# Lornatang/Real_ESRGAN-PyTorch

Measured on NVIDIA B200. Metric: x4 RRDBNet LR Mpix/s, higher is better.
Workload: dtype fp16

## Files before the change

include/resr.h:

```cpp
#ifndef RESR_H_
#define RESR_H_

#include <stddef.h>
#include <stdint.h>

#ifdef __cplusplus
extern "C" {
#endif

#define RESR_OK 0
#define RESR_E_INVALID 1
#define RESR_E_CUDA 2
#define RESR_E_NOMEM 3

int resr_version(void);
const char* resr_last_error(void);

typedef struct resr_generator resr_generator_t;

int resr_generator_create(resr_generator_t** out, int in_channels, int out_channels, int upscale_factor);
void resr_generator_destroy(resr_generator_t* g);

size_t resr_generator_num_params(void);
int resr_generator_num_tensors(void);
int resr_generator_tensor_span(int index, size_t* offset, size_t* count);

int resr_generator_load_params(resr_generator_t* g, const float* flat_params, void* stream);

size_t resr_generator_workspace_bytes(int n, int h, int w);
int resr_generator_set_precision(resr_generator_t* g, int precision);
size_t resr_generator_workspace_bytes_for(const resr_generator_t* g, int n, int h, int w);

int resr_generator_forward(resr_generator_t* g, const float* x, float* y, int n, int h, int w, void* workspace,
                           size_t workspace_bytes, void* stream);

int resr_generator_forward_u8(resr_generator_t* g, const unsigned char* x_u8, unsigned char* y_u8, int n, int h, int w,
                              void* workspace, size_t workspace_bytes, void* stream);
int resr_generator_forward_u8_host(resr_generator_t* g, const unsigned char* x_u8_host, unsigned char* y_u8_host, int n, int h, int w,
                                   void* workspace, size_t workspace_bytes, void* stream);
int resr_tensor_to_image_u8(const float* x, unsigned char* out_hwc, int c, int h, int w, int range_norm, int half, void* stream);

int resr_generator_forward_host(resr_generator_t* g, const float* x_host, float* y_host, int n, int h, int w,
                                void* workspace, size_t workspace_bytes, void* stream);

int resr_generator_forward_host_async(resr_generator_t* g, const float* x_host, float* y_host, int n, int h, int w,
                                      void* workspace, size_t workspace_bytes, void* stream);
int resr_generator_host_sync(resr_generator_t* g);

int resr_generator_launches_per_forward(void);
int resr_set_conv_pair_policy(int policy);
int resr_debug_wait_profile(unsigned long long* out16_host, int reset);

typedef struct resr_conv_desc {
    const void* in16;
    int n, h, w, c_total, cin, cout;
    int fmt_in;
    int mode;
    const float* weight;
    const float* bias;
    int ep_mode;
    int lrelu, clamp01;
    void* out16;
    int out16_fmt, out16_cstride, out16_choff, out16_up2;
    float* outf;
    int outf_cstride, outf_choff;
    const void* res1;
    const void* res2;
    int res_cstride, res_choff;
    int res16, res16_fmt;
    float* out_nchw;
    int out_nchw_c;
    int dbg_flags;
    unsigned long long* dbg;
} resr_conv_desc;
int resr_conv3x3(const resr_conv_desc* d, void* stream);

int resr_nchw_to_nhwc16(const float* x, void* out16, int n, int c, int h, int w, int c_pad, int fmt, void* stream);


int resr_filter2d(const float* image, const float* kernel, float* out, int b, int c, int h, int w, int k,
                  int kernel_batch, void* stream);

size_t resr_usm_workspace_bytes(int b, int c, int h, int w);
int resr_usm_sharp(const float* image, float* out, int b, int c, int h, int w, int radius, int sigma, float weight,
                   float threshold, void* workspace, size_t workspace_bytes, void* stream);
size_t resr_usm_backward_workspace_bytes(int b, int c, int h, int w);
int resr_usm_sharp_backward(const float* image, const float* grad_out, float* grad_in, int b, int c, int h, int w,
                            int radius, int sigma, float weight, float threshold, void* workspace,
                            size_t workspace_bytes, void* stream);

int resr_resize(const float* image, float* out, int planes, int h_in, int w_in, int h_out, int w_out, int mode,
                double scale_h, double scale_w, void* stream);

int resr_gaussian_noise_apply(const float* image, float* out, const float* sigma, const float* gray,
                              const float* noise_color, const float* noise_gray, int b, int c, int h, int w, int clip,
                              int rounds, void* stream);

size_t resr_poisson_workspace_bytes(int b);
int resr_unique_count_u8(const float* image, int* counts_color, int* counts_gray, int b, int c, int h, int w,
                         void* workspace, size_t workspace_bytes, void* stream);
int resr_poisson_rates(const float* image, float* rate_color, float* rate_gray, int b, int c, int h, int w,
                       void* workspace, size_t workspace_bytes, void* stream);
int resr_poisson_noise_apply(const float* image, float* out, const float* scale, const float* gray,
                             const float* samples_color, const float* samples_gray, int b, int c, int h, int w, int clip,
                             int rounds, void* workspace, size_t workspace_bytes, int reuse_counts, void* stream);

int resr_gaussian_noise_sampled(const float* image, float* out, const float* sigma, const float* gray, int b, int c, int h, int w,
                                int clip, int rounds, unsigned long long seed, unsigned long long* call_state, void* stream);

int resr_poisson_noise_sampled(const float* image, float* out, const float* scale, const float* gray, int b, int c, int h, int w,
                               int clip, int rounds, unsigned long long seed, unsigned long long* call_counter,
                               void* workspace, size_t workspace_bytes, void* stream);

int resr_jpeg(const float* image, float* out, const float* quality, float* factor_out, int b, int h, int w,
              int clamp_input, float* q_y, float* q_cb, float* q_cr, void* stream);

int resr_augment_batch_u8(const unsigned char* images_bgr_hwc, float* out_rgb_nchw, const int* ops, int b, int h, int w,
                          void* stream);

int resr_crop(const float* image, float* out, int planes, int h_in, int w_in, int top, int left, int h_out, int w_out,
              int round_to_u8, void* stream);

typedef struct resr_kernel_params {
    int type, kernel_size, isotropic, reserved;
    double sigma_x, sigma_y, theta, beta, cutoff;
} resr_kernel_params;
int resr_synthesize_kernels(const resr_kernel_params* params_host, int count, int pad, double* out_f64, float* out_f32,
                            void* stream);
int resr_synthesize_kernels_device(const resr_kernel_params* params_dev, int count, int kmax, int pad, double* out_f64,
                                   float* out_f32, void* stream);
typedef struct resr_kernel_draw_config {
    int n_sizes, sizes[16];
    int sinc_size_split;
    int final_size;
    double sinc_prob1, sinc_prob2, sinc_prob3;
    double prob1[6], prob2[6];
    double sigma_range1[2], sigma_range2[2];
    double gen_beta_range1[2], gen_beta_range2[2], plateau_beta_range1[2], plateau_beta_range2[2];
} resr_kernel_draw_config;
int resr_draw_degradation_kernel_params(const resr_kernel_draw_config* cfg, int batch, unsigned long long seed,
                                        unsigned long long* call_state, resr_kernel_params* params_dev, void* stream);

size_t resr_generator_train_workspace_bytes(int n, int h, int w);
int resr_generator_forward_train(resr_generator_t* g, const float* x, float* y, int n, int h, int w, void* workspace,
                                 size_t workspace_bytes, void* stream);
int resr_generator_backward_l1(resr_generator_t* g, const float* hr, float* grads_flat, float* loss_out, int n, int h,
                               int w, void* workspace, size_t workspace_bytes, void* stream);
int resr_generator_train_step_l1(resr_generator_t* g, const float* x, const float* hr, float* y, float* grads_flat,
                                 float* loss_out, int n, int h, int w, void* workspace, size_t workspace_bytes,
                                 void* stream);
int resr_generator_step_is_graph(resr_generator_t* g);
int resr_generator_grad_buckets(size_t* offsets, int max_entries);
int resr_generator_wait_grad_bucket(resr_generator_t* g, int bucket, void* stream);
int resr_generator_backward(resr_generator_t* g, const float* dy, float* grads_flat, int n, int h, int w, void* workspace,
                            size_t workspace_bytes, void* stream);

size_t resr_conv3x3_wgrad_workspace_bytes(int n, int h, int w, int cin, int cout);
int resr_conv3x3_wgrad(const void* x16, int x_cstride, int fmt_x, const void* dy16_bf16, int n, int h, int w, int cin,
                       int cout, float* dw, float* db, void* workspace, size_t workspace_bytes, void* stream);

size_t resr_conv3x3_wgrad_nhwc_workspace_bytes(void);
int resr_conv3x3_wgrad_nhwc(const void* x_bf16, int x_cstride, const void* dy_bf16, int dy_cstride, int n, int h, int w,
                            int cin, int cout, float* dw, float* db, void* workspace, size_t workspace_bytes, void* stream);

int resr_niqe_num_blocks(int h, int w, int crop_border, int block);
size_t resr_niqe_workspace_bytes(int b, int h, int w, int crop_border, int block);
int resr_niqe_features(const float* image_rgb, double* features, int b, int h, int w, int crop_border, int block,
                       void* workspace, size_t workspace_bytes, void* stream);

typedef struct resr_resize_spec {
    int mode;
    int out_h, out_w;
    double scale;
} resr_resize_spec;
typedef struct resr_noise_spec {
    int type;
    const float* param;
    const float* gray;
    int gray_any;
    const float* draws_color;
    const float* draws_gray;
    unsigned long long seed;
} resr_noise_spec;
typedef struct resr_degrade_plan {
    int batch, hr_h, hr_w;
    int usm_radius, usm_sigma;
    float usm_weight, usm_threshold;
    int blur1, blur2, final_order;
    int kernel_size, sinc_batched;
    resr_resize_spec resize1, resize2, resize3;
    resr_noise_spec noise1, noise2;
    const float* jpeg1_quality;
    const float* jpeg2_quality;
    int crop_top, crop_left, image_size, upscale;
    unsigned long long* rng_state;
} resr_degrade_plan;
size_t resr_degrade_workspace_bytes(const resr_degrade_plan* plan);
int resr_degrade_batch(const resr_degrade_plan* plan, const float* hr, const float* kernel1, const float* kernel2,
                       const float* sinc_kernel, float* lr_out, float* hr_out, void* workspace, size_t workspace_bytes,
                       void* stream);

int resr_adam_ema_step(float* params, const float* grads, float* exp_avg, float* exp_avg_sq, float* ema_shadow, size_t n,
                       float lr, float beta1, float beta2, float eps, long long step, float ema_decay, float grad_scale,
                       void* stream);

#ifdef __cplusplus
}
#endif
#endif
```

real_esrgan-pytorch_b200/_lib.py:

```python
import ctypes
import os
from ctypes import POINTER, Structure, c_char_p, c_double, c_float, c_int, c_size_t, c_void_p

_HERE = os.path.dirname(os.path.abspath(__file__))
LIB_PATH = os.environ.get("RESR_LIB_PATH") or os.path.join(_HERE, "lib", "libresr.so")


class ResrError(RuntimeError):
    pass


class ConvDesc(Structure):
    _fields_ = [
        ("in16", c_void_p),
        ("n", c_int), ("h", c_int), ("w", c_int), ("c_total", c_int), ("cin", c_int), ("cout", c_int),
        ("fmt_in", c_int), ("mode", c_int),
        ("weight", c_void_p), ("bias", c_void_p),
        ("ep_mode", c_int), ("lrelu", c_int), ("clamp01", c_int),
        ("out16", c_void_p),
        ("out16_fmt", c_int), ("out16_cstride", c_int), ("out16_choff", c_int), ("out16_up2", c_int),
        ("outf", c_void_p),
        ("outf_cstride", c_int), ("outf_choff", c_int),
        ("res1", c_void_p), ("res2", c_void_p),
        ("res_cstride", c_int), ("res_choff", c_int),
        ("res16", c_int), ("res16_fmt", c_int),
        ("out_nchw", c_void_p),
        ("out_nchw_c", c_int),
        ("dbg_flags", c_int),
        ("dbg", c_void_p),
    ]


class ResizeSpec(Structure):
    _fields_ = [("mode", c_int), ("out_h", c_int), ("out_w", c_int), ("scale", c_double)]


class NoiseSpec(Structure):
    _fields_ = [("type", c_int), ("param", c_void_p), ("gray", c_void_p), ("gray_any", c_int), ("draws_color", c_void_p),
                ("draws_gray", c_void_p), ("seed", ctypes.c_ulonglong)]


class DegradePlan(Structure):
    _fields_ = [("batch", c_int), ("hr_h", c_int), ("hr_w", c_int),
                ("usm_radius", c_int), ("usm_sigma", c_int), ("usm_weight", c_float), ("usm_threshold", c_float),
                ("blur1", c_int), ("blur2", c_int), ("final_order", c_int), ("kernel_size", c_int), ("sinc_batched", c_int),
                ("resize1", ResizeSpec), ("resize2", ResizeSpec), ("resize3", ResizeSpec),
                ("noise1", NoiseSpec), ("noise2", NoiseSpec),
                ("jpeg1_quality", c_void_p), ("jpeg2_quality", c_void_p),
                ("crop_top", c_int), ("crop_left", c_int), ("image_size", c_int), ("upscale", c_int),
                ("rng_state", c_void_p)]


class KernelParams(Structure):
    _fields_ = [("type", c_int), ("kernel_size", c_int), ("isotropic", c_int), ("reserved", c_int),
                ("sigma_x", c_double), ("sigma_y", c_double), ("theta", c_double), ("beta", c_double),
                ("cutoff", c_double)]


class KernelDrawConfig(Structure):
    _fields_ = [("n_sizes", c_int), ("sizes", c_int * 16), ("sinc_size_split", c_int), ("final_size", c_int),
                ("sinc_prob1", c_double), ("sinc_prob2", c_double), ("sinc_prob3", c_double),
                ("prob1", c_double * 6), ("prob2", c_double * 6),
                ("sigma_range1", c_double * 2), ("sigma_range2", c_double * 2),
                ("gen_beta_range1", c_double * 2), ("gen_beta_range2", c_double * 2),
                ("plateau_beta_range1", c_double * 2), ("plateau_beta_range2", c_double * 2)]


SIGNATURES = {
    "resr_version": (c_int, []),
    "resr_last_error": (c_char_p, []),
    "resr_generator_create": (c_int, [POINTER(c_void_p), c_int, c_int, c_int]),
    "resr_generator_destroy": (None, [c_void_p]),
    "resr_generator_num_params": (c_size_t, []),
    "resr_generator_num_tensors": (c_int, []),
    "resr_generator_tensor_span": (c_int, [c_int, POINTER(c_size_t), POINTER(c_size_t)]),
    "resr_generator_load_params": (c_int, [c_void_p, c_void_p, c_void_p]),
    "resr_generator_workspace_bytes": (c_size_t, [c_int, c_int, c_int]),
    "resr_generator_workspace_bytes_for": (c_size_t, [c_void_p, c_int, c_int, c_int]),
    "resr_generator_set_precision": (c_int, [c_void_p, c_int]),
    "resr_generator_forward": (c_int, [c_void_p, c_void_p, c_void_p, c_int, c_int, c_int, c_void_p, c_size_t, c_void_p]),
    "resr_generator_forward_u8": (c_int, [c_void_p, c_void_p, c_void_p, c_int, c_int, c_int, c_void_p, c_size_t, c_void_p]),
    "resr_generator_forward_u8_host": (c_int, [c_void_p, c_void_p, c_void_p, c_int, c_int, c_int, c_void_p, c_size_t, c_void_p]),
    "resr_tensor_to_image_u8": (c_int, [c_void_p, c_void_p, c_int, c_int, c_int, c_int, c_int, c_void_p]),
    "resr_generator_forward_host": (c_int, [c_void_p, c_void_p, c_void_p, c_int, c_int, c_int, c_void_p, c_size_t, c_void_p]),
    "resr_generator_forward_host_async": (c_int, [c_void_p, c_void_p, c_void_p, c_int, c_int, c_int, c_void_p, c_size_t, c_void_p]),
    "resr_generator_host_sync": (c_int, [c_void_p]),
    "resr_generator_launches_per_forward": (c_int, []),
    "resr_debug_wait_profile": (c_int, [c_void_p, c_int]),
    "resr_set_conv_pair_policy": (c_int, [c_int]),
    "resr_conv3x3": (c_int, [POINTER(ConvDesc), c_void_p]),
    "resr_nchw_to_nhwc16": (c_int, [c_void_p, c_void_p, c_int, c_int, c_int, c_int, c_int, c_int, c_void_p]),
    "resr_filter2d": (c_int, [c_void_p, c_void_p, c_void_p, c_int, c_int, c_int, c_int, c_int, c_int, c_void_p]),
    "resr_usm_workspace_bytes": (c_size_t, [c_int, c_int, c_int, c_int]),
    "resr_niqe_num_blocks": (c_int, [c_int, c_int, c_int, c_int]),
    "resr_niqe_workspace_bytes": (c_size_t, [c_int, c_int, c_int, c_int, c_int]),
    "resr_niqe_features": (c_int, [c_void_p, c_void_p, c_int, c_int, c_int, c_int, c_int, c_void_p, c_size_t, c_void_p]),
    "resr_augment_batch_u8": (c_int, [c_void_p, c_void_p, c_void_p, c_int, c_int, c_int, c_void_p]),
    "resr_usm_backward_workspace_bytes": (c_size_t, [c_int, c_int, c_int, c_int]),
    "resr_usm_sharp_backward": (c_int, [c_void_p, c_void_p, c_void_p, c_int, c_int, c_int, c_int, c_int, c_int, c_float, c_float,
                                        c_void_p, c_size_t, c_void_p]),
    "resr_usm_sharp": (c_int, [c_void_p, c_void_p, c_int, c_int, c_int, c_int, c_int, c_int, c_float, c_float, c_void_p,
                               c_size_t, c_void_p]),
    "resr_resize": (c_int, [c_void_p, c_void_p, c_int, c_int, c_int, c_int, c_int, c_int, c_double, c_double, c_void_p]),
    "resr_gaussian_noise_apply": (c_int, [c_void_p, c_void_p, c_void_p, c_void_p, c_void_p, c_void_p, c_int, c_int, c_int,
                                          c_int, c_int, c_int, c_void_p]),
    "resr_poisson_workspace_bytes": (c_size_t, [c_int]),
    "resr_unique_count_u8": (c_int, [c_void_p, c_void_p, c_void_p, c_int, c_int, c_int, c_int, c_void_p, c_size_t, c_void_p]),
    "resr_poisson_rates": (c_int, [c_void_p, c_void_p, c_void_p, c_int, c_int, c_int, c_int, c_void_p, c_size_t, c_void_p]),
    "resr_poisson_noise_apply": (c_int, [c_void_p, c_void_p, c_void_p, c_void_p, c_void_p, c_void_p, c_int, c_int, c_int,
                                         c_int, c_int, c_int, c_void_p, c_size_t, c_int, c_void_p]),
    "resr_gaussian_noise_sampled": (c_int, [c_void_p, c_void_p, c_void_p, c_void_p, c_int, c_int, c_int, c_int, c_int, c_int,
                                            ctypes.c_ulonglong, c_void_p, c_void_p]),
    "resr_poisson_noise_sampled": (c_int, [c_void_p, c_void_p, c_void_p, c_void_p, c_int, c_int, c_int, c_int, c_int, c_int,
                                           ctypes.c_ulonglong, c_void_p, c_void_p, c_size_t, c_void_p]),
    "resr_jpeg": (c_int, [c_void_p, c_void_p, c_void_p, c_void_p, c_int, c_int, c_int, c_int, c_void_p, c_void_p, c_void_p,
                          c_void_p]),
    "resr_degrade_workspace_bytes": (c_size_t, [POINTER(DegradePlan)]),
    "resr_degrade_batch": (c_int, [POINTER(DegradePlan), c_void_p, c_void_p, c_void_p, c_void_p, c_void_p, c_void_p, c_void_p,
                                   c_size_t, c_void_p]),
    "resr_adam_ema_step": (c_int, [c_void_p, c_void_p, c_void_p, c_void_p, c_void_p, c_size_t, c_float, c_float, c_float,
                                   c_float, ctypes.c_longlong, c_float, c_float, c_void_p]),
    "resr_synthesize_kernels": (c_int, [POINTER(KernelParams), c_int, c_int, c_void_p, c_void_p, c_void_p]),
    "resr_synthesize_kernels_device": (c_int, [c_void_p, c_int, c_int, c_int, c_void_p, c_void_p, c_void_p]),
    "resr_draw_degradation_kernel_params": (c_int, [POINTER(KernelDrawConfig), c_int, ctypes.c_ulonglong, c_void_p, c_void_p, c_void_p]),
    "resr_generator_train_workspace_bytes": (c_size_t, [c_int, c_int, c_int]),
    "resr_generator_forward_train": (c_int, [c_void_p, c_void_p, c_void_p, c_int, c_int, c_int, c_void_p, c_size_t, c_void_p]),
    "resr_generator_backward_l1": (c_int, [c_void_p, c_void_p, c_void_p, c_void_p, c_int, c_int, c_int, c_void_p, c_size_t,
                                           c_void_p]),
    "resr_generator_train_step_l1": (c_int, [c_void_p, c_void_p, c_void_p, c_void_p, c_void_p, c_void_p, c_int, c_int, c_int,
                                             c_void_p, c_size_t, c_void_p]),
    "resr_generator_step_is_graph": (c_int, [c_void_p]),
    "resr_generator_backward": (c_int, [c_void_p, c_void_p, c_void_p, c_int, c_int, c_int, c_void_p, c_size_t, c_void_p]),
    "resr_conv3x3_wgrad_workspace_bytes": (c_size_t, [c_int, c_int, c_int, c_int, c_int]),
    "resr_generator_grad_buckets": (c_int, [c_void_p, c_int]),
    "resr_generator_wait_grad_bucket": (c_int, [c_void_p, c_int, c_void_p]),
    "resr_conv3x3_wgrad_nhwc_workspace_bytes": (c_size_t, []),
    "resr_conv3x3_wgrad_nhwc": (c_int, [c_void_p, c_int, c_void_p, c_int, c_int, c_int, c_int, c_int, c_int, c_void_p, c_void_p,
                                        c_void_p, c_size_t, c_void_p]),
    "resr_conv3x3_wgrad": (c_int, [c_void_p, c_int, c_int, c_void_p, c_int, c_int, c_int, c_int, c_int, c_void_p, c_void_p,
                                   c_void_p, c_size_t, c_void_p]),
    "resr_crop": (c_int, [c_void_p, c_void_p, c_int, c_int, c_int, c_int, c_int, c_int, c_int, c_int, c_void_p]),
}

_lib = None


def lib():
    global _lib
    if _lib is None:
        if not os.path.exists(LIB_PATH):
            raise ResrError(
                f"{LIB_PATH} is missing: build it with `make` (or `python -c 'import __graft_entry__ as g; g.build()'`). "
                "resr_b200 has no CPU / PyTorch fallback.")
        handle = ctypes.CDLL(LIB_PATH)
        for name, (res, args) in SIGNATURES.items():
            fn = getattr(handle, name)
            fn.restype = res
            fn.argtypes = args
        _lib = handle
    return _lib


def check(rc):
    if rc != 0:
        msg = lib().resr_last_error()
        raise ResrError(f"libresr error {rc}: {msg.decode() if msg else '?'}")


def stream_ptr(device=None):
    import torch
    return c_void_p(torch.cuda.current_stream(device).cuda_stream)


def ptr(t):
    if t is None:
        return c_void_p(0)
    return c_void_p(t.data_ptr())
```

real_esrgan-pytorch_b200/csrc/conv3x3.cuh:

```cuda
#pragma once
#include <cstdint>
#include <cuda.h>
#include <cuda_runtime.h>

namespace resr {

enum EpMode : int {
    EP_PLAIN = 0,
    EP_RDB = 1,
    EP_RRDB = 2,
    EP_SKIP = 3,
    EP_ADD2 = 4,
};

struct ConvArgs {
    int N, H, W;
    int BW, BN;
    int nxs;
    int ncg;
    int nchunks;
    int tail_ksteps;
    int mode;
    int nstages;
    int nepi;
    int reverse;
    int epi_bufs;
    int fmt_in;
    long long rows_total;
    long long rows_total_pair;
    const uint8_t* wpack;
    const float* bias;
    int ep_mode, lrelu, clamp01;
    int has_out16;
    int out16_fmt;
    int out16_choff;
    int out16_up2;
    int has_outf;
    int outf_choff;
    float* outf;
    int outf_cstride;
    int has_res1;
    int res_choff;
    const void* res1;
    int res1_cstride;
    int res16;
    int res16_fmt;
    const void* res2;
    int res2_cstride;
    float* out_nchw;
    int out_nchw_c;
    unsigned char* out_u8;
    unsigned slice_nores_mask;
    unsigned slice_noutf_mask;
    unsigned slice_no16_mask;
    int out16_slice_fixed;
    const void* mask16;
    int mask16_cstride, mask16_choff;
    float res2_scale;
    float out16_scale;
    float* out_nchw_raw;
    int dbg_flags;
    unsigned long long* dbg;
};

inline int conv3x3_tail_ksteps(int cin) {
#ifdef RESR_NO_TAILSKIP
    (void)cin;
    return 4;
#else
    const int r = cin % 64;
    return r == 0 || r > 32 ? 4 : (r > 16 ? 2 : 1);
#endif
}

struct ConvMaps {
    CUtensorMap a;
    CUtensorMap o16;
    CUtensorMap of;
};

cudaError_t conv3x3_launch(const ConvMaps& maps, const ConvArgs& args, int cout_slice, int nslices, int num_sms,
                           cudaStream_t stream);

bool conv3x3_plan_smem(ConvArgs* args, int cout_slice);

bool conv3x3_pair_plan_smem(ConvArgs* args, int nout);
cudaError_t conv3x3_pair_launch(const ConvMaps& maps, const ConvArgs& args, int nout, int nslices, int num_sms,
                                cudaStream_t stream);

int conv3x3_wait_profile(unsigned long long* out16, int reset);

struct ConvLaunchCfg {
    int pair;
    int nout;
    int nslices;
};
int conv3x3_set_pair_policy(int policy);
bool conv3x3_choose(ConvArgs* args, int pack_nout, int pack_nslices, ConvLaunchCfg* cfg);
cudaError_t conv3x3_run(const ConvMaps& maps, const ConvArgs& args, const ConvLaunchCfg& cfg, int num_sms, cudaStream_t stream);

int conv3x3_make_tmap_act(CUtensorMap* out, const void* base, int N, int H, int W, int C, int mode, int BW, int BN,
                          int cvalid = 0);
int conv3x3_make_tmap_out16(CUtensorMap* out, const void* base, int N, int H, int W, int C, int nout, int BW, int BN,
                            int up2);
int conv3x3_make_tmap_f32(CUtensorMap* out, const void* base, int N, int H, int W, int C, int BW, int BN);

void conv3x3_pick_tile(int W, int* BW, int* BN);

}
```

real_esrgan-pytorch_b200/csrc/conv3x3_pair.cu:

```cuda
#include <cuda_bf16.h>
#include <cuda_fp16.h>

#include <cstdlib>
#include <cstring>

#include "conv3x3.cuh"
#include "device_state.h"
#include "ptx.cuh"

namespace resr {

__device__ unsigned long long g_wait_prof[16];
#ifdef RESR_PROFILE_WAITS
#define PROF_DECL(name) long long name = 0
#define PROF_T0(t) const long long t = clock64()
#define PROF_ADD(acc, t) acc += clock64() - t
#define PROF_FLUSH(idx, v) do { if ((threadIdx.x & 31) == 0) atomicAdd(&g_wait_prof[idx], static_cast<unsigned long long>(v)); } while (0)
#else
#define PROF_DECL(name)
#define PROF_T0(t)
#define PROF_ADD(acc, t)
#define PROF_FLUSH(idx, v)
#endif

namespace {

constexpr int kStageBytes = 17408;
constexpr int kMaxStages = 12;
constexpr int kMiscBytes = 1024;
constexpr int kSmemMax = 232448;
constexpr int kTileFBytes = 16384;

struct RowRange {
    int g0, g1;
};

constexpr uint32_t kDescHi = (1024u >> 4) | (1u << 14) | (2u << 29);
__device__ __forceinline__ uint64_t desc_of(uint32_t lo) { return (static_cast<uint64_t>(kDescHi) << 32) | lo; }

__host__ __device__ inline int epi_buf_bytes_pair(const ConvArgs& a, int subw) {
    const int f = a.has_outf ? kTileFBytes : 0;
    const int h = a.has_out16 ? 128 * subw * 2 : 0;
    return f + (h + 1023) / 1024 * 1024;
}
__host__ __device__ inline int epi_group_bytes_pair(const ConvArgs& a, int subw) {
    return (a.epi_bufs == 2 ? 2 : 1) * epi_buf_bytes_pair(a, subw);
}

template <int S>
__device__ __forceinline__ uint32_t ring_slot(uint32_t v) { return (S - v % S) % S; }
template <int S>
__device__ __forceinline__ uint32_t ring_parity(uint32_t v) { return (v / S) & 1u; }

__device__ __forceinline__ void unpack16x8(const uint4 q, int fmt, float (&f)[8]) {
    const uint32_t w4[4] = {q.x, q.y, q.z, q.w};
#pragma unroll
    for (int i = 0; i < 4; ++i) {
        if (fmt == 1) {
            f[2 * i] = __uint_as_float(w4[i] << 16);
            f[2 * i + 1] = __uint_as_float(w4[i] & 0xFFFF0000u);
        } else {
            const float2 h = __half22float2(*reinterpret_cast<const __half2*>(&w4[i]));
            f[2 * i] = h.x;
            f[2 * i + 1] = h.y;
        }
    }
}

template <int NOUT, int KS, int I0, int I1>
__device__ __forceinline__ void issue_range(uint32_t d0, uint32_t a_lo, uint32_t b_lo, uint32_t idesc) {
    constexpr uint32_t WT = (3 * NOUT / 2 * 128) >> 4;
#pragma unroll
    for (int i = I0; i < I1; ++i) {
        const int dx = i / KS, ks = i % KS;
        umma2_f16(d0, desc_of(a_lo + dx * 8 + ks * 2), desc_of(b_lo + dx * WT + ks * 2), idesc, 1);
    }
}

template <int NOUT, int NDX, int HALF>
__device__ __forceinline__ void issue_half(int ks, uint32_t d0, uint32_t a_lo, uint32_t b_lo, uint32_t idesc) {
#define RESR_HALF(KS)                                                                       \
    if (HALF == 0) issue_range<NOUT, KS, 0, (NDX * KS) / 2>(d0, a_lo, b_lo, idesc);          \
    else issue_range<NOUT, KS, (NDX * KS) / 2, NDX * KS>(d0, a_lo, b_lo, idesc)
    if (ks == 2) { RESR_HALF(2); }
    else if (ks == 1) { RESR_HALF(1); }
    else { RESR_HALF(4); }
#undef RESR_HALF
}

template <int NOUT, int MODE, int S>
__device__ __forceinline__ void mma_role(const ConvArgs& a, const RowRange rr, const uint32_t tbase, const uint32_t wsm_addr,
                                         const uint32_t stg_addr, const uint32_t full_a, const uint32_t empty_a,
                                         const uint32_t accfull_a, const uint32_t slotfree_a) {
    constexpr uint32_t WT = (3 * NOUT / 2 * 128) >> 4;
    const uint32_t idesc = make_idesc_f16(a.fmt_in, 256, 3 * NOUT);
    const uint32_t w_lo = (wsm_addr & 0x3FFFFu) >> 4;
    const uint32_t s_lo = (stg_addr & 0x3FFFFu) >> 4;
    const int nsteps = MODE == 0 ? a.nchunks : a.nchunks * 3;
    const uint32_t b_step = (MODE == 0 ? 3 : 1) * WT;
    const int nstages = a.nstages;
    const int H = a.H;
    int stage = 0;
    uint32_t phase = 0;
    uint32_t a_lo = s_lo;
    int pending_empty = -1;
    bool full_ready = false, slot_ready = false;
    uint32_t vnew = 1;
    uint32_t acq = 0;
    PROF_DECL(p_full); PROF_DECL(p_slot); PROF_DECL(p_steps);
    PROF_T0(p_t0);
    for (int g = rr.g0; g < rr.g1;) {
        const int ya = g % H;
        const int yb = min(H, ya + (rr.g1 - g));
        const int ra = max(ya - 1, 0), rb = min(yb, H - 1);
        vnew += 1;
        for (int r = ra; r <= rb; ++r, ++vnew) {
            if (slot_ready && acq == vnew) {
                ++acq;
            } else {
                PROF_T0(p_t);
                while (static_cast<int>(vnew - acq) >= 0) {
                    mbar_wait_a(slotfree_a + (ring_slot<S>(acq) << 3), ring_parity<S>(acq));
                    ++acq;
                }
                PROF_ADD(p_slot, p_t);
            }
            slot_ready = false;
            tc_fence_after();
            const uint32_t s0 = ring_slot<S>(vnew), s1 = ring_slot<S>(vnew - 1), s2 = ring_slot<S>(vnew - 2);
            const uint32_t d0 = tbase + s0 * NOUT;
            uint32_t b_lo = w_lo;
            for (int st = 0; st < nsteps; ++st, b_lo += b_step) {
                if (!full_ready) { PROF_T0(p_t); mbar_wait_a(full_a + (stage << 3), phase); PROF_ADD(p_full, p_t); }
                tc_fence_after();
#ifdef RESR_PROFILE_WAITS
                ++p_steps;
#endif
                const bool last = (st == nsteps - 1);
                const int ks = (st >= nsteps - (MODE == 0 ? 1 : 3)) ? a.tail_ksteps : 4;
                if (elect_one()) {
                    issue_half<NOUT, MODE == 0 ? 3 : 1, 0>(ks, d0, a_lo, b_lo, idesc);
                    if (pending_empty >= 0) umma2_commit_mc(empty_a + (pending_empty << 3), 3);
                }
                __syncwarp();
                pending_empty = stage;
                const uint32_t a_cur = a_lo;
                if (++stage == nstages) { stage = 0; phase ^= 1u; a_lo = s_lo; } else { a_lo += kStageBytes >> 4; }
                full_ready = mbar_test_wait_a(full_a + (stage << 3), phase);
                if (last && r < rb) slot_ready = mbar_test_wait_a(slotfree_a + (ring_slot<S>(vnew + 1) << 3), ring_parity<S>(vnew + 1));
                if (elect_one()) {
                    issue_half<NOUT, MODE == 0 ? 3 : 1, 1>(ks, d0, a_cur, b_lo, idesc);
                    if (last) {
                        umma2_commit_mc(accfull_a + (s2 << 3), 3);
                        if (r == rb) {
                            umma2_commit_mc(accfull_a + (s1 << 3), 3);
                            umma2_commit_mc(accfull_a + (s0 << 3), 3);
                        }
                    }
                }
                __syncwarp();
            }
        }
        vnew += 1;
        g += yb - ya;
    }
    if (pending_empty >= 0) {
        if (elect_one()) umma2_commit_mc(empty_a + (pending_empty << 3), 3);
        __syncwarp();
    }
#ifdef RESR_PROFILE_WAITS
    PROF_FLUSH(0, clock64() - p_t0); PROF_FLUSH(1, p_full); PROF_FLUSH(2, p_slot); PROF_FLUSH(3, p_steps);
#endif
}

template <int W>
__device__ __forceinline__ void tmem_ld_w(uint32_t taddr, float* v) {
    if (W == 32) tmem_ld32(taddr, v); else tmem_ld16(taddr, v);
}
template <int W>
__device__ __forceinline__ void tmem_zero_w(uint32_t taddr) {
    if (W == 32) tmem_st_zero32(taddr); else tmem_st_zero16(taddr);
}
template <int W>
__device__ __forceinline__ void tmem_init_bias(uint32_t taddr, const float* __restrict__ bias_w) {
    float b[W];
#pragma unroll
    for (int i = 0; i < W / 4; ++i) {
        const float4 q = reinterpret_cast<const float4*>(bias_w)[i];
        b[4 * i] = q.x; b[4 * i + 1] = q.y; b[4 * i + 2] = q.z; b[4 * i + 3] = q.w;
    }
    if (W == 32) tmem_st32(taddr, b); else tmem_st16(taddr, b);
}

}

template <int NOUT>
__global__ void __launch_bounds__(512, 1)
conv3x3_pair_kernel(const __grid_constant__ CUtensorMap tmapA, const __grid_constant__ CUtensorMap tmapO16,
                    const __grid_constant__ CUtensorMap tmapOF, const ConvArgs a) {
    constexpr int NT = 3 * NOUT;
    constexpr int NH = NT / 2;
    constexpr int WHALF = NH * 128;
    constexpr int NSUB = NOUT == 64 ? 2 : 1;
    constexpr int SUBW = NOUT / NSUB;
    constexpr int SLOTS = NOUT == 64 ? 8 : 16;
    constexpr int S = SLOTS - 2;
    extern __shared__ uint8_t smem_raw[];
    uint8_t* smem = smem_raw + ((1024u - (smem_u32(smem_raw) & 1023u)) & 1023u);

    const int warp = __shfl_sync(0xffffffffu, threadIdx.x >> 5, 0);
    const int lane = threadIdx.x & 31;
    const int slice = blockIdx.y;
    const uint32_t rank = cluster_ctarank();
    const uint32_t wbytes = static_cast<uint32_t>(a.nchunks) * 3u * WHALF;
    const int epi_bytes = epi_group_bytes_pair(a, SUBW);

    uint8_t* wsm = smem;
    uint8_t* stg = smem + wbytes;
    uint8_t* epi = stg + a.nstages * kStageBytes;
    uint8_t* misc = epi + a.nepi * epi_bytes;
    uint64_t* full = reinterpret_cast<uint64_t*>(misc);
    uint64_t* empty = full + kMaxStages;
    uint64_t* acc_full = empty + kMaxStages;
    uint64_t* slot_free = acc_full + 16;
    uint64_t* wbar = slot_free + 16;
    uint64_t* wpair = wbar + 1;
    uint32_t* tmem_ptr = reinterpret_cast<uint32_t*>(wpair + 1);
    float* bias_s = reinterpret_cast<float*>(misc + 512);

    if (threadIdx.x == 0) {
        prefetch_tmap(&tmapA);
        if (a.has_out16) prefetch_tmap(&tmapO16);
        if (a.has_outf) prefetch_tmap(&tmapOF);
        for (int i = 0; i < a.nstages; ++i) {
            mbar_init(full + i, 1);
            mbar_init(empty + i, 1);
        }
        for (int i = 0; i < S; ++i) {
            mbar_init(acc_full + i, 1);
            mbar_init(slot_free + i, 8);
        }
        mbar_init(wbar, 1);
        mbar_init(wpair, 2);
        fence_mbar_init();
    }
    if (warp == 2) {
        tmem_alloc2(tmem_ptr, 512);
        tmem_relinquish2();
    }
    if (threadIdx.x >= 128 && threadIdx.x < 128 + NOUT) bias_s[threadIdx.x - 128] = a.bias[slice * NOUT + threadIdx.x - 128];
    tc_fence_before();
    __syncthreads();
    cluster_sync_all();
    tc_fence_after();
    const uint32_t tbase = *tmem_ptr;
    grid_dep_launch();

    RowRange rr;
    {
        const unsigned npairs = gridDim.x >> 1, pidx = blockIdx.x >> 1, rows = static_cast<unsigned>(a.rows_total_pair);
        rr.g0 = static_cast<int>(rows * pidx / npairs);
        rr.g1 = static_cast<int>(rows * (pidx + 1) / npairs);
    }
    const int H = a.H;

    if (warp == 0) {
        if (elect_one()) {
            mbar_expect_tx(wbar, wbytes);
            constexpr int G = NOUT == 64 ? 32 : NOUT / 2;
            constexpr int BPD = NOUT / G;
            constexpr int NB = 3 * BPD / 2;
            for (int c = 0; c < a.nchunks; ++c) {
                for (int dx = 0; dx < 3; ++dx) {
                    uint8_t* dst = wsm + (c * 3 + dx) * WHALF;
#pragma unroll
                    for (int j = 0; j < NB; ++j) {
                        const int blk = static_cast<int>(rank) * NB + j;
                        const int dyv = blk / BPD, part = blk % BPD;
                        const int dy = a.reverse ? 2 - dyv : dyv;
                        const uint8_t* src;
                        if (NOUT == 64)
                            src = a.wpack + ((static_cast<size_t>(slice * 2 + part) * a.nchunks + c) * 3 + dx) * (96 * 128) +
                                  static_cast<size_t>(dy) * 32 * 128;
                        else
                            src = a.wpack + ((static_cast<size_t>(slice) * a.nchunks + c) * 3 + dx) * (NT * 128) +
                                  static_cast<size_t>(dy * NOUT + part * G) * 128;
                        bulk_load_1d(dst + j * G * 128, src, G * 128, wbar);
                    }
                }
            }
        }
        __syncwarp();
        grid_dep_wait();
        int stage = 0;
        uint32_t phase = 0;
        const int ndx = a.mode == 0 ? 1 : 3;
        const uint32_t tx_bytes = a.mode == 0 ? (a.BW + 2) * 128 : 128 * 128;
        const uint32_t full0 = map_to_cta(smem_u32(full), 0);
        PROF_DECL(p_empty);
        PROF_T0(p_t0);
        const int ncg2 = (a.ncg + 1) >> 1;
        for (int g = rr.g0; g < rr.g1;) {
            const int cg2 = g / H;
            const int cg = 2 * (a.reverse ? ncg2 - 1 - cg2 : cg2) + static_cast<int>(rank);
            const int ya = g % H;
            const int yb = min(H, ya + (rr.g1 - g));
            const int n0 = (cg / a.nxs) * a.BN;
            const int x0 = (cg % a.nxs) * a.BW;
            const int ra = max(ya - 1, 0), rb = min(yb, H - 1);
            for (int r = ra; r <= rb; ++r) {
                for (int c = 0; c < a.nchunks; ++c) {
                    for (int dx = 0; dx < ndx; ++dx) {
                        { PROF_T0(p_t); mbar_wait(empty + stage, phase ^ 1); PROF_ADD(p_empty, p_t); }
                        if (elect_one()) {
                            if (rank == 0) mbar_expect_tx(full + stage, 2 * tx_bytes);
                            tma_load_4d_pair(stg + stage * kStageBytes, &tmapA, full0 + (stage << 3), c * 64,
                                             a.mode == 0 ? x0 - 1 : x0 + dx - 1, a.reverse ? H - 1 - r : r, n0);
                        }
                        __syncwarp();
                        if (++stage == a.nstages) { stage = 0; phase ^= 1; }
                    }
                }
            }
            g += yb - ya;
        }
#ifdef RESR_PROFILE_WAITS
        PROF_FLUSH(4, clock64() - p_t0); PROF_FLUSH(5, p_empty);
#endif
    } else if (warp == 1) {
        mbar_wait(wbar, 0);
        if (elect_one()) mbar_arrive_cluster(map_to_cta(smem_u32(wpair), 0));
        __syncwarp();
        if (rank == 0) {
            mbar_wait(wpair, 0);
            tc_fence_after();
            if (a.mode == 0) mma_role<NOUT, 0, S>(a, rr, tbase, smem_u32(wsm), smem_u32(stg), smem_u32(full), smem_u32(empty), smem_u32(acc_full), smem_u32(slot_free));
            else mma_role<NOUT, 1, S>(a, rr, tbase, smem_u32(wsm), smem_u32(stg), smem_u32(full), smem_u32(empty), smem_u32(acc_full), smem_u32(slot_free));
        }
    } else if (warp >= 4) {
        const int gi = (warp - 4) >> 2;
        const int q = warp & 3;
        const int m = q * 32 + lane;
        const bool lead_warp = ((warp - 4) & 3) == 0;
        uint8_t* const tile_base = epi + gi * epi_bytes;
        const int buf_bytes = epi_buf_bytes_pair(a, SUBW);
        const bool two_bufs = a.epi_bufs == 2;
        uint32_t pass = 0;
        const uint32_t lane_base = tbase + (static_cast<uint32_t>(q * 32) << 16);
        const uint32_t free0 = map_to_cta(smem_u32(slot_free), 0);
        const int img_in_tile = m / a.BW;
        const int x_in_tile = m % a.BW;
        {
            const int s_lo = gi * S / a.nepi, s_hi = (gi + 1) * S / a.nepi;
            for (int s = s_lo; s < s_hi; ++s) {
#pragma unroll
                for (int c = 0; c < NOUT; c += SUBW) {
                    tmem_init_bias<SUBW>(lane_base + s * NOUT + c, bias_s + c);
                    if (s < 2) tmem_zero_w<SUBW>(lane_base + (S + s) * NOUT + c);
                }
            }
            tmem_st_wait();
            tc_fence_before();
            __syncwarp();
            if (lane == 0)
                for (int s = s_lo; s < s_hi; ++s) mbar_arrive_cluster(free0 + (s << 3));
        }
        grid_dep_wait();
        PROF_DECL(p_acc); PROF_DECL(p_tile); PROF_DECL(p_drain); PROF_DECL(p_math); PROF_DECL(p_store); PROF_DECL(p_rows);
        PROF_T0(p_t0);
        uint32_t v0 = 0;
        const int ncg2 = (a.ncg + 1) >> 1;
        for (int g = rr.g0; g < rr.g1;) {
            const int cg2 = g / H;
            const int cg = 2 * (a.reverse ? ncg2 - 1 - cg2 : cg2) + static_cast<int>(rank);
            const int ya = g % H;
            const int yb = min(H, ya + (rr.g1 - g));
            const int n0 = (cg / a.nxs) * a.BN;
            const int x0 = (cg % a.nxs) * a.BW;
            const int n = n0 + img_in_tile;
            const int x = x0 + x_in_tile;
            const bool valid = (n < a.N) && (x < a.W);
            const int ra = max(ya - 1, 0), rb = min(yb, H - 1);
            const int n_acc = rb - ra + 3;
            for (int j = 0; j < n_acc; ++j) {
                const uint32_t v = v0 + j;
                if (static_cast<int>(v % a.nepi) != gi) continue;
                const int yv = ra - 1 + j;
                const bool emit = (yv >= ya) && (yv < yb);
                const int y = a.reverse ? H - 1 - yv : yv;
                const uint32_t slot = ring_slot<S>(v);
                const uint32_t col = slot * NOUT;
                const uint32_t col2 = (S + slot) * NOUT;
                const bool dual = slot < 2;
                const size_t pix = (static_cast<size_t>(valid ? n : 0) * a.H + y) * a.W + (valid ? x : 0);
                bool waited = false;
#pragma unroll 1
                for (int h = 0; h < NSUB; ++h) {
                    const int ls = slice * NSUB + h;
                    const bool use_res1 = a.has_res1 && !((a.slice_nores_mask >> ls) & 1u);
                    const bool use_outf = a.has_outf && !((a.slice_noutf_mask >> ls) & 1u);
                    const bool use_o16 = a.has_out16 && !((a.slice_no16_mask >> ls) & 1u);
                    const bool staged = use_o16 || use_outf;
                    float4 resv[SUBW / 4];
                    if (emit && use_res1) {
                        if (a.res16) {
                            const uint4* rp = reinterpret_cast<const uint4*>(static_cast<const uint16_t*>(a.res1) + pix * a.res1_cstride +
                                                                             a.res_choff + ls * SUBW);
#pragma unroll
                            for (int i = 0; i < SUBW / 8; ++i) {
                                const uint4 q4 = rp[i];
                                resv[i] = make_float4(__uint_as_float(q4.x), __uint_as_float(q4.y), __uint_as_float(q4.z), __uint_as_float(q4.w));
                            }
                        } else {
                            const float4* rp = reinterpret_cast<const float4*>(static_cast<const float*>(a.res1) + pix * a.res1_cstride +
                                                                               a.res_choff + ls * SUBW);
#pragma unroll
                            for (int i = 0; i < SUBW / 4; ++i) resv[i] = rp[i];
                        }
                    }
                    if (!waited) {
                        PROF_T0(p_t);
                        mbar_wait(acc_full + slot, ring_parity<S>(v));
                        PROF_ADD(p_acc, p_t);
                        tc_fence_after();
                        waited = true;
                    }
                    float val[SUBW];
                    PROF_T0(p_td);
                    tmem_ld_w<SUBW>(lane_base + col + h * SUBW, val);
                    if (dual) {
                        float val2[SUBW];
                        tmem_ld_w<SUBW>(lane_base + col2 + h * SUBW, val2);
                        tmem_ld_wait();
#pragma unroll
                        for (int i = 0; i < SUBW; ++i) val[i] = __fadd_rn(val[i], val2[i]);
                        tmem_zero_w<SUBW>(lane_base + col2 + h * SUBW);
                    } else {
                        tmem_ld_wait();
                    }
                    tmem_init_bias<SUBW>(lane_base + col + h * SUBW, bias_s + h * SUBW);
                    if (h == NSUB - 1) {
                        tmem_st_wait();
                        tc_fence_before();
                        __syncwarp();
                        if (lane == 0) mbar_arrive_cluster(free0 + (slot << 3));
                    }
                    PROF_ADD(p_drain, p_td);
                    if (!emit) continue;
                    PROF_T0(p_tm);
#ifdef RESR_PROFILE_WAITS
                    ++p_rows;
#endif

                    if (use_res1 && a.res16) {
                        float wide[SUBW];
#pragma unroll
                        for (int i = 0; i < SUBW / 8; ++i) {
                            float f8[8];
                            unpack16x8(make_uint4(__float_as_uint(resv[i].x), __float_as_uint(resv[i].y), __float_as_uint(resv[i].z),
                                                  __float_as_uint(resv[i].w)), a.res16_fmt, f8);
#pragma unroll
                            for (int e = 0; e < 8; ++e) wide[8 * i + e] = f8[e];
                        }
#pragma unroll
                        for (int i = 0; i < SUBW / 4; ++i) resv[i] = make_float4(wide[4 * i], wide[4 * i + 1], wide[4 * i + 2], wide[4 * i + 3]);
                    }
                    if (use_res1) {
#pragma unroll
                        for (int i = 0; i < SUBW / 4; ++i) {
                            const float4 r4 = resv[i];
                            if (a.ep_mode == EP_SKIP || a.ep_mode == EP_ADD2) {
                                val[4 * i + 0] = __fadd_rn(r4.x, val[4 * i + 0]);
                                val[4 * i + 1] = __fadd_rn(r4.y, val[4 * i + 1]);
                                val[4 * i + 2] = __fadd_rn(r4.z, val[4 * i + 2]);
                                val[4 * i + 3] = __fadd_rn(r4.w, val[4 * i + 3]);
                            } else {
                                const float2 p01 = __fmul2_rn(make_float2(val[4 * i + 0], val[4 * i + 1]), make_float2(0.2f, 0.2f));
                                const float2 p23 = __fmul2_rn(make_float2(val[4 * i + 2], val[4 * i + 3]), make_float2(0.2f, 0.2f));
                                const float2 s01 = __fadd2_rn(p01, make_float2(r4.x, r4.y));
                                const float2 s23 = __fadd2_rn(p23, make_float2(r4.z, r4.w));
                                val[4 * i + 0] = s01.x; val[4 * i + 1] = s01.y; val[4 * i + 2] = s23.x; val[4 * i + 3] = s23.y;
                            }
                        }
                    }
                    PROF_ADD(p_math, p_tm);
                    uint8_t* const tileR = tile_base + ((two_bufs && (pass & 1u)) ? buf_bytes : 0);
                    uint8_t* const tile16 = tileR + (a.has_outf ? kTileFBytes : 0);
                    if (staged) {
                        PROF_T0(p_t);
                        if (lead_warp) { if (two_bufs) tma_store_wait_read1(); else tma_store_wait_read(); }
                        named_bar_sync(1 + gi, 128);
                        PROF_ADD(p_tile, p_t);
                        ++pass;
                    }
                    PROF_T0(p_ts);
                    if (a.ep_mode == EP_RRDB) {
                        if (a.res16) {
                            const uint4* r2 = reinterpret_cast<const uint4*>(static_cast<const uint16_t*>(a.res2) + pix * a.res2_cstride +
                                                                             a.res_choff + ls * SUBW);
#pragma unroll
                            for (int i = 0; i < SUBW / 8; ++i) {
                                float f8[8];
                                unpack16x8(r2[i], a.res16_fmt, f8);
#pragma unroll
                                for (int e = 0; e < 8; e += 2) {
                                    const float2 pp = __fmul2_rn(make_float2(val[8 * i + e], val[8 * i + e + 1]), make_float2(0.2f, 0.2f));
                                    const float2 ss = __fadd2_rn(pp, make_float2(f8[e], f8[e + 1]));
                                    val[8 * i + e] = ss.x; val[8 * i + e + 1] = ss.y;
                                }
                            }
                        } else {
                            const float4* r2 = reinterpret_cast<const float4*>(static_cast<const float*>(a.res2) + pix * a.res2_cstride +
                                                                               a.res_choff + ls * SUBW);
#pragma unroll
                            for (int i = 0; i < SUBW / 4; ++i) {
                                const float4 r4 = __ldg(r2 + i);
                                val[4 * i + 0] = __fadd_rn(__fmul_rn(val[4 * i + 0], 0.2f), r4.x);
                                val[4 * i + 1] = __fadd_rn(__fmul_rn(val[4 * i + 1], 0.2f), r4.y);
                                val[4 * i + 2] = __fadd_rn(__fmul_rn(val[4 * i + 2], 0.2f), r4.z);
                                val[4 * i + 3] = __fadd_rn(__fmul_rn(val[4 * i + 3], 0.2f), r4.w);
                            }
                        }
                    }
                    if (a.ep_mode == EP_ADD2 && a.res2) {
                        const float4* r2 = reinterpret_cast<const float4*>(static_cast<const float*>(a.res2) + pix * a.res2_cstride + a.res_choff + ls * SUBW);
#pragma unroll
                        for (int i = 0; i < SUBW / 4; ++i) {
                            const float4 r4 = __ldg(r2 + i);
                            val[4 * i + 0] = fmaf(a.res2_scale, r4.x, val[4 * i + 0]);
                            val[4 * i + 1] = fmaf(a.res2_scale, r4.y, val[4 * i + 1]);
                            val[4 * i + 2] = fmaf(a.res2_scale, r4.z, val[4 * i + 2]);
                            val[4 * i + 3] = fmaf(a.res2_scale, r4.w, val[4 * i + 3]);
                        }
                    }
                    if (a.lrelu) {
#pragma unroll
                        for (int i = 0; i < SUBW / 2; ++i) {
                            const float2 t = __fmul2_rn(make_float2(val[2 * i], val[2 * i + 1]), make_float2(0.2f, 0.2f));
                            val[2 * i] = fmaxf(val[2 * i], t.x);
                            val[2 * i + 1] = fmaxf(val[2 * i + 1], t.y);
                        }
                    }
                    if (a.out_nchw_raw && valid) {
                        const size_t plane = static_cast<size_t>(a.H) * a.W;
                        float* o = a.out_nchw_raw + static_cast<size_t>(n) * a.out_nchw_c * plane + static_cast<size_t>(y) * a.W + x;
#pragma unroll
                        for (int c = 0; c < SUBW; ++c) {
                            const int cc = ls * SUBW + c;
                            if (cc < a.out_nchw_c) o[static_cast<size_t>(cc) * plane] = val[c];
                        }
                    }
                    if (a.clamp01) {
#pragma unroll
                        for (int i = 0; i < SUBW; ++i) val[i] = fminf(fmaxf(val[i], 0.f), 1.f);
                    }
                    if (use_outf) {
#pragma unroll
                        for (int i = 0; i < SUBW / 4; ++i)
                            *reinterpret_cast<float4*>(tileR + m * 128 + ((i ^ (m & 7)) << 4)) =
                                make_float4(val[4 * i], val[4 * i + 1], val[4 * i + 2], val[4 * i + 3]);
                    }
                    if (use_o16 && a.mask16) {
                        const uint4* mk = reinterpret_cast<const uint4*>(static_cast<const uint16_t*>(a.mask16) + pix * a.mask16_cstride +
                                                                         a.mask16_choff + ls * SUBW);
#pragma unroll
                        for (int i = 0; i < SUBW / 8; ++i) {
                            const uint4 q4 = __ldg(mk + i);
                            const uint32_t w4[4] = {q4.x, q4.y, q4.z, q4.w};
#pragma unroll
                            for (int e = 0; e < 8; ++e) {
                                const uint32_t h16 = (w4[e >> 1] >> ((e & 1) * 16)) & 0xFFFFu;
                                const bool pos = ((h16 & 0x8000u) == 0) && ((h16 & 0x7FFFu) != 0);
                                if (!pos) val[8 * i + e] = __fmul_rn(val[8 * i + e], 0.2f);
                            }
                        }
                    }
                    if (use_o16 && a.out16_scale != 0.f) {
#pragma unroll
                        for (int i = 0; i < SUBW; ++i) val[i] = __fmul_rn(val[i], a.out16_scale);
                    }
                    if (use_o16) {
                        uint32_t pk[SUBW / 2];
#pragma unroll
                        for (int i = 0; i < SUBW / 2; ++i) {
                            if (a.out16_fmt == 1) {
                                __nv_bfloat162 hh = __floats2bfloat162_rn(val[2 * i], val[2 * i + 1]);
                                pk[i] = *reinterpret_cast<uint32_t*>(&hh);
                            } else {
                                pk[i] = pack_f16x2_sat(val[2 * i], val[2 * i + 1]);
                            }
                        }
                        uint4* dst = reinterpret_cast<uint4*>(tile16 + m * (SUBW * 2));
#pragma unroll
                        for (int i = 0; i < SUBW / 8; ++i) dst[i] = make_uint4(pk[4 * i], pk[4 * i + 1], pk[4 * i + 2], pk[4 * i + 3]);
                    }
                    if (staged) {
                        fence_proxy_async_smem();
                        named_bar_sync(1 + gi, 128);
                        if (lead_warp) {
                            if (elect_one()) {
                                if (use_outf) tma_store_4d(&tmapOF, tileR, a.outf_choff + ls * SUBW, x0, y, n0);
                                if (use_o16) {
                                    const int c0 = a.out16_choff + (a.out16_slice_fixed ? 0 : ls * SUBW);
                                    if (!a.out16_up2) {
                                        tma_store_4d(&tmapO16, tile16, c0, x0, y, n0);
                                    } else {
#pragma unroll
                                        for (int s = 0; s < 4; ++s) tma_store_5d(&tmapO16, tile16, c0, s & 1, x0, 2 * y + (s >> 1), n0);
                                    }
                                }
                                tma_store_commit();
                            }
                            __syncwarp();
                        }
                    }
                    PROF_ADD(p_store, p_ts);
                    if (a.out_nchw && valid) {
                        const size_t plane = static_cast<size_t>(a.H) * a.W;
                        float* o = a.out_nchw + static_cast<size_t>(n) * a.out_nchw_c * plane + static_cast<size_t>(y) * a.W + x;
#pragma unroll
                        for (int c = 0; c < SUBW; ++c) {
                            const int cc = ls * SUBW + c;
                            if (cc < a.out_nchw_c) o[static_cast<size_t>(cc) * plane] = val[c];
                        }
                    }
                    if (a.out_u8 && valid) {
                        unsigned char* o = a.out_u8 + ((static_cast<size_t>(n) * a.H + y) * a.W + x) * a.out_nchw_c;
#pragma unroll
                        for (int c = 0; c < SUBW; ++c) {
                            const int cc = ls * SUBW + c;
                            if (cc < a.out_nchw_c) o[cc] = static_cast<unsigned char>(fminf(fmaxf(__fmul_rn(val[c], 255.f), 0.f), 255.f));
                        }
                    }
                }
            }
            v0 += n_acc;
            g += yb - ya;
        }
        if (lead_warp) tma_store_wait_all();
#ifdef RESR_PROFILE_WAITS
        if (warp == 4) {
            PROF_FLUSH(6, clock64() - p_t0); PROF_FLUSH(7, p_acc); PROF_FLUSH(8, p_tile);
            PROF_FLUSH(9, p_drain); PROF_FLUSH(10, p_math); PROF_FLUSH(11, p_store); PROF_FLUSH(12, p_rows);
        }
#endif
    }

    tc_fence_before();
    cluster_sync_all();
    if (warp == 2) tmem_dealloc2(tbase, 512);
}


bool conv3x3_pair_plan_smem(ConvArgs* a, int nout) {
    const int subw = nout == 64 ? 32 : nout;
    const int wbytes = a->nchunks * 3 * (3 * nout / 2) * 128;
    int nepi = a->has_outf ? 2 : 3;
    const char* env = getenv("RESR_CONV_NEPI");
    if (env) nepi = atoi(env);
    if (nepi < 1) nepi = 1;
    if (nepi > 3) nepi = 3;
    static const int env_bufs = getenv("RESR_CONV_EPI_BUFS") ? atoi(getenv("RESR_CONV_EPI_BUFS")) : 2;
    for (;; --nepi) {
        a->nepi = nepi;
        for (int bufs = env_bufs == 2 ? 2 : 1; bufs >= 1; --bufs) {
            a->epi_bufs = bufs;
            const int fixed = 1024 + wbytes + nepi * epi_group_bytes_pair(*a, subw) + kMiscBytes;
            int ns = (kSmemMax - fixed) / kStageBytes;
            if (ns > kMaxStages) ns = kMaxStages;
            if ((bufs == 2 && ns >= 6) || (bufs == 1 && (ns >= 4 || nepi == 1))) {
                a->nstages = ns;
                return ns >= 2;
            }
        }
    }
}

template <int NOUT>
static cudaError_t launch_pair_t(const ConvMaps& maps, const ConvArgs& args, dim3 grid, int threads, cudaStream_t stream) {
    static PerDevice<bool> attr;
    if (!attr.cur()) {
        cudaError_t e = cudaFuncSetAttribute(conv3x3_pair_kernel<NOUT>, cudaFuncAttributeMaxDynamicSharedMemorySize, kSmemMax);
        if (e != cudaSuccess) return e;
        attr.cur() = true;
    }
    cudaLaunchConfig_t cfg;
    memset(&cfg, 0, sizeof(cfg));
    cfg.gridDim = grid;
    cfg.blockDim = dim3(threads, 1, 1);
    cfg.dynamicSmemBytes = kSmemMax;
    cfg.stream = stream;
    cudaLaunchAttribute at[2];
    at[0].id = cudaLaunchAttributeProgrammaticStreamSerialization;
    at[0].val.programmaticStreamSerializationAllowed = 1;
    at[1].id = cudaLaunchAttributeClusterDimension;
    at[1].val.clusterDim.x = 2;
    at[1].val.clusterDim.y = 1;
    at[1].val.clusterDim.z = 1;
    cfg.attrs = at;
    cfg.numAttrs = 2;
    return cudaLaunchKernelEx(&cfg, conv3x3_pair_kernel<NOUT>, maps.a, maps.o16, maps.of, args);
}

cudaError_t conv3x3_pair_launch(const ConvMaps& maps, const ConvArgs& args_in, int nout, int nslices, int num_sms,
                                cudaStream_t stream) {
    ConvArgs args = args_in;
    const int subw = nout == 64 ? 32 : nout;
    const int wbytes = args.nchunks * 3 * (3 * nout / 2) * 128;
    const int smem = 1024 + wbytes + args.nstages * kStageBytes + args.nepi * epi_group_bytes_pair(args, subw) + kMiscBytes;
    if (args.nstages < 2 || args.nepi < 1 || args.nepi > 3 || smem > kSmemMax) return cudaErrorInvalidConfiguration;
    if (args.has_outf && subw != 32) return cudaErrorInvalidConfiguration;
    const long long ncg2 = (args.ncg + 1) / 2;
    args.rows_total_pair = ncg2 * args.H;
    long long npairs = (num_sms / 2) / nslices;
    const long long min_rows = 4;
    const long long cap = (args.rows_total_pair + min_rows - 1) / min_rows;
    if (npairs > cap) npairs = cap;
    if (npairs < 1) npairs = 1;
    if (args.rows_total_pair * (npairs + 1) >= (1ll << 31)) return cudaErrorInvalidValue;
    if (args.tail_ksteps != 1 && args.tail_ksteps != 2 && args.tail_ksteps != 4) args.tail_ksteps = 4;
    const dim3 grid(static_cast<unsigned>(2 * npairs), static_cast<unsigned>(nslices), 1);
    const int threads = 128 + 128 * args.nepi;
    if (nout == 64) return launch_pair_t<64>(maps, args, grid, threads, stream);
    if (nout == 32) return launch_pair_t<32>(maps, args, grid, threads, stream);
    if (nout == 16) return launch_pair_t<16>(maps, args, grid, threads, stream);
    return cudaErrorInvalidValue;
}

int conv3x3_wait_profile(unsigned long long* out16, int reset) {
    if (out16 && cudaMemcpyFromSymbol(out16, g_wait_prof, sizeof(unsigned long long) * 16) != cudaSuccess) return -1;
    if (reset) {
        unsigned long long z[16] = {0};
        if (cudaMemcpyToSymbol(g_wait_prof, z, sizeof(z)) != cudaSuccess) return -1;
    }
    return 0;
}

static int g_pair_policy = -1;
int conv3x3_set_pair_policy(int policy) {
    if (g_pair_policy < 0) g_pair_policy = getenv("RESR_CONV_PAIR") ? atoi(getenv("RESR_CONV_PAIR")) : 1;
    const int prev = g_pair_policy;
    if (policy >= 0 && policy <= 2) g_pair_policy = policy;
    return prev;
}

bool conv3x3_choose(ConvArgs* a, int pack_nout, int pack_nslices, ConvLaunchCfg* cfg) {
    const int env_pair = conv3x3_set_pair_policy(-1);
    static const int env_n64 = getenv("RESR_CONV_PAIR_N64") ? atoi(getenv("RESR_CONV_PAIR_N64")) : 1;
    cfg->pair = 0;
    cfg->nout = pack_nout;
    cfg->nslices = pack_nslices;
    const long long pair_rows = static_cast<long long>((a->ncg + 1) / 2) * a->H;
    const bool big_enough = pair_rows >= 6 * 74 || env_pair == 2;
    if (env_pair && a->ncg >= 2 && big_enough) {
        ConvArgs t = *a;
        int nout = pack_nout, nslices = pack_nslices;
        if (env_n64 && pack_nout == 32 && pack_nslices % 2 == 0) { nout = 64; nslices = pack_nslices / 2; }
        if (conv3x3_pair_plan_smem(&t, nout)) {
            *a = t;
            cfg->pair = 1; cfg->nout = nout; cfg->nslices = nslices;
            return true;
        }
    }
    return conv3x3_plan_smem(a, pack_nout);
}

cudaError_t conv3x3_run(const ConvMaps& maps, const ConvArgs& args, const ConvLaunchCfg& cfg, int num_sms, cudaStream_t stream) {
    if (cfg.pair) return conv3x3_pair_launch(maps, args, cfg.nout, cfg.nslices, num_sms, stream);
    return conv3x3_launch(maps, args, cfg.nout, cfg.nslices, num_sms, stream);
}

}
```

real_esrgan-pytorch_b200/csrc/conv3x3_tc.cu:

```cuda
#include <cuda_bf16.h>
#include <cuda_fp16.h>

#include <cstdlib>
#include <cstring>

#include "conv3x3.cuh"
#include "device_state.h"
#include "ptx.cuh"

#ifdef RESR_EXPERIMENTS
#define DBGF(x) ((a.dbg_flags & (x)) != 0)
#else
#define DBGF(x) false
#endif

namespace resr {

static constexpr int kStageBytes = 17408;
static constexpr int kMaxStages = 12;
static constexpr int kSlots = 16;
static constexpr int kMiscBytes = 1024;
static constexpr int kSmemMax = 232448;
static constexpr int kTileFBytes = 16384;

struct RowRange {
    int g0, g1;
};

__device__ __forceinline__ RowRange cta_rows(const ConvArgs& a) {
    RowRange r;
    const unsigned rows = static_cast<unsigned>(a.rows_total);
    r.g0 = static_cast<int>(rows * blockIdx.x / gridDim.x);
    r.g1 = static_cast<int>(rows * (blockIdx.x + 1) / gridDim.x);
    return r;
}

__device__ __forceinline__ unsigned long long gtimer() {
    unsigned long long t;
    asm volatile("mov.u64 %0, %globaltimer;" : "=l"(t));
    return t;
}
#define RESR_DBG(slot) do { if (a.dbg && blockIdx.x == 0 && blockIdx.y == 0 && (threadIdx.x & 31) == 0) a.dbg[slot] = gtimer(); } while (0)

__device__ __forceinline__ uint32_t slot_of(uint32_t v) { return (16u - (v & 15u)) & 15u; }

__host__ __device__ inline int epi_group_bytes(const ConvArgs& a, int nout) {
    const int f = a.has_outf ? kTileFBytes : 0;
    const int h = a.has_out16 ? 128 * nout * 2 : 0;
    return f + (h + 1023) / 1024 * 1024;
}


static constexpr uint32_t kDescHi = (1024u >> 4) | (1u << 14) | (2u << 29);
__device__ __forceinline__ uint64_t desc_of(uint32_t lo) { return (static_cast<uint64_t>(kDescHi) << 32) | lo; }

template <int NOUT, int SPLIT, int KS, int I0, int I1>
__device__ __forceinline__ void issue_range(uint32_t d0, uint32_t ring0, uint32_t a_lo, uint32_t b_lo, uint32_t idesc3,
                                            uint32_t idesc2, uint32_t idesc1) {
    constexpr uint32_t WT = (3 * NOUT * 128) >> 4;
    constexpr uint32_t ROWS = (NOUT * 128) >> 4;
#pragma unroll
    for (int i = I0; i < I1; ++i) {
        const int dx = i / KS, ks = i % KS;
        const uint64_t ad = desc_of(a_lo + dx * 8 + ks * 2);
        const uint32_t bl = b_lo + dx * WT + ks * 2;
        if (SPLIT == 0) {
            umma_f16(d0, ad, desc_of(bl), idesc3, 1);
        } else if (SPLIT == 1) {
            umma_f16(d0, ad, desc_of(bl), idesc2, 1);
            umma_f16(ring0, ad, desc_of(bl + 2 * ROWS), idesc1, 1);
        } else {
            umma_f16(d0, ad, desc_of(bl), idesc1, 1);
            umma_f16(ring0, ad, desc_of(bl + ROWS), idesc2, 1);
        }
    }
}
template <int NOUT, int KS, int I0, int I1>
__device__ __forceinline__ void issue_part(uint32_t s0, uint32_t d0, uint32_t ring0, uint32_t a_lo, uint32_t b_lo,
                                           uint32_t idesc3, uint32_t idesc2, uint32_t idesc1) {
    if (s0 <= 13) issue_range<NOUT, 0, KS, I0, I1>(d0, ring0, a_lo, b_lo, idesc3, idesc2, idesc1);
    else if (s0 == 14) issue_range<NOUT, 1, KS, I0, I1>(d0, ring0, a_lo, b_lo, idesc3, idesc2, idesc1);
    else issue_range<NOUT, 2, KS, I0, I1>(d0, ring0, a_lo, b_lo, idesc3, idesc2, idesc1);
}


template <int NOUT, int NDX, int HALF>
__device__ __forceinline__ void issue_half(int ks, uint32_t s0, uint32_t d0, uint32_t ring0, uint32_t a_lo, uint32_t b_lo,
                                           uint32_t idesc3, uint32_t idesc2, uint32_t idesc1) {
#define RESR_HALF(KS)                                                                                              \
    if (HALF == 0) issue_part<NOUT, KS, 0, (NDX * KS) / 2>(s0, d0, ring0, a_lo, b_lo, idesc3, idesc2, idesc1);       \
    else issue_part<NOUT, KS, (NDX * KS) / 2, NDX * KS>(s0, d0, ring0, a_lo, b_lo, idesc3, idesc2, idesc1)
    if (ks == 2) { RESR_HALF(2); }
    else if (ks == 1) { RESR_HALF(1); }
    else { RESR_HALF(4); }
#undef RESR_HALF
}

template <int W>
__device__ __forceinline__ void tmem_init_bias_w(uint32_t taddr, const float* __restrict__ bias_w) {
    float b[W];
#pragma unroll
    for (int i = 0; i < W / 4; ++i) {
        const float4 q = reinterpret_cast<const float4*>(bias_w)[i];
        b[4 * i] = q.x; b[4 * i + 1] = q.y; b[4 * i + 2] = q.z; b[4 * i + 3] = q.w;
    }
    if (W == 32) tmem_st32(taddr, b); else tmem_st16(taddr, b);
}

__device__ __forceinline__ void unpack16x8(const uint4 q, int fmt, float (&f)[8]) {
    const uint32_t w4[4] = {q.x, q.y, q.z, q.w};
#pragma unroll
    for (int i = 0; i < 4; ++i) {
        if (fmt == 1) {
            f[2 * i] = __uint_as_float(w4[i] << 16);
            f[2 * i + 1] = __uint_as_float(w4[i] & 0xFFFF0000u);
        } else {
            const float2 h = __half22float2(*reinterpret_cast<const __half2*>(&w4[i]));
            f[2 * i] = h.x;
            f[2 * i + 1] = h.y;
        }
    }
}

template <int NOUT, int MODE>
__device__ __forceinline__ void mma_role(const ConvArgs& a, const RowRange rr, const uint32_t tbase, const uint32_t wsm_addr,
                                         const uint32_t stg_addr, const uint32_t full_a, const uint32_t empty_a,
                                         const uint32_t accfull_a, const uint32_t slotfree_a) {
    constexpr uint32_t WT = (3 * NOUT * 128) >> 4;
    const uint32_t idesc3 = make_idesc_f16(a.fmt_in, 128, 3 * NOUT);
    const uint32_t idesc2 = make_idesc_f16(a.fmt_in, 128, 2 * NOUT);
    const uint32_t idesc1 = make_idesc_f16(a.fmt_in, 128, NOUT);
    const uint32_t w_lo = (wsm_addr & 0x3FFFFu) >> 4;
    const uint32_t s_lo = (stg_addr & 0x3FFFFu) >> 4;
    const int nsteps = MODE == 0 ? a.nchunks : a.nchunks * 3;
    const uint32_t b_step = (MODE == 0 ? 3 : 1) * WT;
    const int nstages = a.nstages;
    const int H = a.H;
    const bool dbg_quarter = DBGF(4), dbg_nomma = DBGF(16);
    int stage = 0;
    uint32_t phase = 0;
    uint32_t a_lo = s_lo;
    int pending_empty = -1;
    bool full_ready = false, slot_ready = false;
    uint32_t vnew = 1;
    uint32_t acq = 0;
    for (int g = rr.g0; g < rr.g1;) {
        const int ya = g % H;
        const int yb = min(H, ya + (rr.g1 - g));
        const int ra = max(ya - 1, 0), rb = min(yb, H - 1);
        vnew += 1;
        for (int r = ra; r <= rb; ++r, ++vnew) {
            if (slot_ready && acq == vnew) {
                ++acq;
            } else {
                while (static_cast<int>(vnew - acq) >= 0) {
                    mbar_wait_a(slotfree_a + (((0u - acq) & 15u) << 3), (acq >> 4) & 1u);
                    ++acq;
                }
            }
            slot_ready = false;
            tc_fence_after();
            const uint32_t s0 = (0u - vnew) & 15u;
            const uint32_t d0 = tbase + s0 * NOUT;
            uint32_t b_lo = w_lo;
            for (int st = 0; st < nsteps; ++st, b_lo += b_step) {
                if (!full_ready) mbar_wait_a(full_a + (stage << 3), phase);
                tc_fence_after();
                const bool last = (st == nsteps - 1);
                const int ks = dbg_quarter ? 1 : ((st >= nsteps - (MODE == 0 ? 1 : 3)) ? a.tail_ksteps : 4);
                if (elect_one()) {
                    if (!dbg_nomma) issue_half<NOUT, MODE == 0 ? 3 : 1, 0>(ks, s0, d0, tbase, a_lo, b_lo, idesc3, idesc2, idesc1);
                    if (pending_empty >= 0) umma_commit_a(empty_a + (pending_empty << 3));
                }
                __syncwarp();
                pending_empty = stage;
                const uint32_t a_cur = a_lo;
                if (++stage == nstages) { stage = 0; phase ^= 1u; a_lo = s_lo; } else { a_lo += kStageBytes >> 4; }
                full_ready = mbar_test_wait_a(full_a + (stage << 3), phase);
                if (last && r < rb) slot_ready = mbar_test_wait_a(slotfree_a + (((0u - (vnew + 1)) & 15u) << 3), ((vnew + 1) >> 4) & 1u);
                if (elect_one()) {
                    if (!dbg_nomma) issue_half<NOUT, MODE == 0 ? 3 : 1, 1>(ks, s0, d0, tbase, a_cur, b_lo, idesc3, idesc2, idesc1);
                    if (last) {
                        umma_commit_a(accfull_a + (((s0 + 2) & 15u) << 3));
                        if (r == rb) {
                            umma_commit_a(accfull_a + (((s0 + 1) & 15u) << 3));
                            umma_commit_a(accfull_a + (s0 << 3));
                        }
                    }
                }
                __syncwarp();
            }
        }
        vnew += 1;
        g += yb - ya;
    }
    if (pending_empty >= 0) {
        if (elect_one()) umma_commit_a(empty_a + (pending_empty << 3));
        __syncwarp();
    }
}

template <int NOUT>
__global__ void __launch_bounds__(512, 1)
conv3x3_tc_kernel(const __grid_constant__ CUtensorMap tmapA, const __grid_constant__ CUtensorMap tmapO16,
                  const __grid_constant__ CUtensorMap tmapOF,
                  const ConvArgs a) {
    constexpr int NT = 3 * NOUT;
    constexpr int WTILE = NT * 128;
    extern __shared__ uint8_t smem_raw[];
    uint8_t* smem = smem_raw + ((1024u - (smem_u32(smem_raw) & 1023u)) & 1023u);

    const int warp = __shfl_sync(0xffffffffu, threadIdx.x >> 5, 0);
    const int lane = threadIdx.x & 31;
    const int slice = blockIdx.y;
    if (threadIdx.x == 0) RESR_DBG(0);
    const uint32_t wbytes = static_cast<uint32_t>(a.nchunks) * 3u * WTILE;
    const int epi_bytes = epi_group_bytes(a, NOUT);

    uint8_t* wsm = smem;
    uint8_t* stg = smem + wbytes;
    uint8_t* epi = stg + a.nstages * kStageBytes;
    uint8_t* misc = epi + a.nepi * epi_bytes;
    uint64_t* full = reinterpret_cast<uint64_t*>(misc);
    uint64_t* empty = full + kMaxStages;
    uint64_t* acc_full = empty + kMaxStages;
    uint64_t* slot_free = acc_full + kSlots;
    uint64_t* wbar = slot_free + kSlots;
    uint32_t* tmem_ptr = reinterpret_cast<uint32_t*>(wbar + 1);
    float* bias_s = reinterpret_cast<float*>(misc + 512);

    if (threadIdx.x == 0) {
        prefetch_tmap(&tmapA);
        if (a.has_out16) prefetch_tmap(&tmapO16);
        if (a.has_outf) prefetch_tmap(&tmapOF);
        for (int i = 0; i < a.nstages; ++i) {
            mbar_init(full + i, 1);
            mbar_init(empty + i, 1);
        }
        for (int i = 0; i < kSlots; ++i) {
            mbar_init(acc_full + i, 1);
            mbar_init(slot_free + i, 128);
        }
        mbar_init(wbar, 1);
        fence_mbar_init();
    }
    if (warp == 2) {
        tmem_alloc(tmem_ptr, 512);
        tmem_relinquish();
    }
    if (threadIdx.x >= 128 && threadIdx.x < 128 + NOUT) bias_s[threadIdx.x - 128] = a.bias[slice * NOUT + threadIdx.x - 128];
    tc_fence_before();
    __syncthreads();
    tc_fence_after();
    const uint32_t tbase = *tmem_ptr;
    if (threadIdx.x == 0) RESR_DBG(1);
    grid_dep_launch();

    const RowRange rr = cta_rows(a);
    const int H = a.H;

    if (warp == 0) {
        if (elect_one()) {
            mbar_expect_tx(wbar, wbytes);
            const uint8_t* wsrc = a.wpack + static_cast<size_t>(slice) * wbytes;
            for (int c = 0; c < a.nchunks; ++c) bulk_load_1d(wsm + c * 3 * WTILE, wsrc + static_cast<size_t>(c) * 3 * WTILE, 3 * WTILE, wbar);
        }
        __syncwarp();
        grid_dep_wait();
        RESR_DBG(2);
        int stage = 0;
        uint32_t phase = 0;
        const int ndx = a.mode == 0 ? 1 : 3;
        const uint32_t tx_bytes = a.mode == 0 ? (a.BW + 2) * 128 : 128 * 128;
        for (int g = rr.g0; g < rr.g1;) {
            const int cg = g / H;
            const int ya = g % H;
            const int yb = min(H, ya + (rr.g1 - g));
            const int n0 = (cg / a.nxs) * a.BN;
            const int x0 = (cg % a.nxs) * a.BW;
            const int ra = max(ya - 1, 0), rb = min(yb, H - 1);
            for (int r = ra; r <= rb; ++r) {
                for (int c = 0; c < a.nchunks; ++c) {
                    for (int dx = 0; dx < ndx; ++dx) {
                        mbar_wait(empty + stage, phase ^ 1);
                        if (elect_one()) {
                            if (DBGF(32)) {
                                mbar_arrive(full + stage);
                            } else {
                                mbar_expect_tx(full + stage, tx_bytes);
                                tma_load_4d(stg + stage * kStageBytes, &tmapA, full + stage, c * 64,
                                            a.mode == 0 ? x0 - 1 : x0 + dx - 1, DBGF(2) ? 0 : r, DBGF(2) ? 0 : n0);
                            }
                        }
                        __syncwarp();
                        if (++stage == a.nstages) { stage = 0; phase ^= 1; }
                    }
                }
            }
            g += yb - ya;
        }
    } else if (warp == 1) {
        mbar_wait(wbar, 0);
        RESR_DBG(3);
        tc_fence_after();
        if (a.mode == 0) mma_role<NOUT, 0>(a, rr, tbase, smem_u32(wsm), smem_u32(stg), smem_u32(full), smem_u32(empty), smem_u32(acc_full), smem_u32(slot_free));
        else mma_role<NOUT, 1>(a, rr, tbase, smem_u32(wsm), smem_u32(stg), smem_u32(full), smem_u32(empty), smem_u32(acc_full), smem_u32(slot_free));
        RESR_DBG(5);
    } else if (warp >= 4) {
        const int gi = (warp - 4) >> 2;
        const int q = warp & 3;
        const int m = q * 32 + lane;
        const bool lead_warp = ((warp - 4) & 3) == 0;
        const bool use_res1 = a.has_res1 && !((a.slice_nores_mask >> slice) & 1u);
        const bool use_outf = a.has_outf && !((a.slice_noutf_mask >> slice) & 1u);
        const bool use_o16 = a.has_out16 && !((a.slice_no16_mask >> slice) & 1u);
        const bool staged = use_o16 || use_outf;
        uint8_t* tileR = epi + gi * epi_bytes;
        uint8_t* tile16 = tileR + (a.has_outf ? kTileFBytes : 0);
        const uint32_t lane_base = tbase + (static_cast<uint32_t>(q * 32) << 16);
        const int img_in_tile = m / a.BW;
        const int x_in_tile = m % a.BW;
        {
            const int s_lo = gi * kSlots / a.nepi, s_hi = (gi + 1) * kSlots / a.nepi;
            for (int s = s_lo; s < s_hi; ++s) tmem_init_bias_w<NOUT>(lane_base + s * NOUT, bias_s);
            tmem_st_wait();
            tc_fence_before();
            for (int s = s_lo; s < s_hi; ++s) mbar_arrive(slot_free + s);
        }
        grid_dep_wait();
        uint32_t v0 = 0;
        for (int g = rr.g0; g < rr.g1;) {
            const int cg = g / H;
            const int ya = g % H;
            const int yb = min(H, ya + (rr.g1 - g));
            const int n0 = (cg / a.nxs) * a.BN;
            const int x0 = (cg % a.nxs) * a.BW;
            const int n = n0 + img_in_tile;
            const int x = x0 + x_in_tile;
            const bool valid = (n < a.N) && (x < a.W);
            const int ra = max(ya - 1, 0), rb = min(yb, H - 1);
            const int n_acc = rb - ra + 3;
            for (int j = 0; j < n_acc; ++j) {
                const uint32_t v = v0 + j;
                if (static_cast<int>(v % static_cast<uint32_t>(a.nepi)) != gi) continue;
                const int y = ra - 1 + j;
                const bool emit = (y >= ya) && (y < yb) && !DBGF(8);
                const uint32_t slot = slot_of(v);
                float4 resv[NOUT / 4];
                if (emit && use_res1) {
                    const size_t pix = (static_cast<size_t>(valid ? n : 0) * a.H + y) * a.W + (valid ? x : 0);
                    if (a.res16) {
                        const uint4* rp = reinterpret_cast<const uint4*>(static_cast<const uint16_t*>(a.res1) + pix * a.res1_cstride +
                                                                         a.res_choff + slice * NOUT);
#pragma unroll
                        for (int i = 0; i < NOUT / 8; ++i) {
                            const uint4 q4 = rp[i];
                            resv[i] = make_float4(__uint_as_float(q4.x), __uint_as_float(q4.y), __uint_as_float(q4.z), __uint_as_float(q4.w));
                        }
                    } else {
                        const float4* rp = reinterpret_cast<const float4*>(static_cast<const float*>(a.res1) + pix * a.res1_cstride +
                                                                           a.res_choff + slice * NOUT);
#pragma unroll
                        for (int i = 0; i < NOUT / 4; ++i) resv[i] = rp[i];
                    }
                }
                mbar_wait(acc_full + slot, static_cast<uint32_t>(v >> 4) & 1);
                tc_fence_after();
                float val[NOUT];
                if (NOUT == 32) tmem_ld32(lane_base + slot * NOUT, val); else tmem_ld16(lane_base + slot * NOUT, val);
                tmem_ld_wait();
                tmem_init_bias_w<NOUT>(lane_base + slot * NOUT, bias_s);
                tmem_st_wait();
                tc_fence_before();
                mbar_arrive(slot_free + slot);
                if (!emit) continue;

                if (use_res1 && a.res16) {
                    float wide[NOUT];
#pragma unroll
                    for (int i = 0; i < NOUT / 8; ++i) {
                        float f8[8];
                        unpack16x8(make_uint4(__float_as_uint(resv[i].x), __float_as_uint(resv[i].y), __float_as_uint(resv[i].z),
                                              __float_as_uint(resv[i].w)), a.res16_fmt, f8);
#pragma unroll
                        for (int e = 0; e < 8; ++e) wide[8 * i + e] = f8[e];
                    }
#pragma unroll
                    for (int i = 0; i < NOUT / 4; ++i) resv[i] = make_float4(wide[4 * i], wide[4 * i + 1], wide[4 * i + 2], wide[4 * i + 3]);
                }
                if (use_res1) {
#pragma unroll
                    for (int i = 0; i < NOUT / 4; ++i) {
                        const float4 r4 = resv[i];
                        if (a.ep_mode == EP_SKIP || a.ep_mode == EP_ADD2) {
                            val[4 * i + 0] = __fadd_rn(r4.x, val[4 * i + 0]);
                            val[4 * i + 1] = __fadd_rn(r4.y, val[4 * i + 1]);
                            val[4 * i + 2] = __fadd_rn(r4.z, val[4 * i + 2]);
                            val[4 * i + 3] = __fadd_rn(r4.w, val[4 * i + 3]);
                        } else {
                            val[4 * i + 0] = __fadd_rn(__fmul_rn(val[4 * i + 0], 0.2f), r4.x);
                            val[4 * i + 1] = __fadd_rn(__fmul_rn(val[4 * i + 1], 0.2f), r4.y);
                            val[4 * i + 2] = __fadd_rn(__fmul_rn(val[4 * i + 2], 0.2f), r4.z);
                            val[4 * i + 3] = __fadd_rn(__fmul_rn(val[4 * i + 3], 0.2f), r4.w);
                        }
                    }
                }
                if (staged) {
                    if (lead_warp) tma_store_wait_read();
                    named_bar_sync(1 + gi, 128);
                }
                if (a.ep_mode == EP_RRDB) {
                    const size_t pix = (static_cast<size_t>(valid ? n : 0) * a.H + y) * a.W + (valid ? x : 0);
                    if (a.res16) {
                        const uint4* r2 = reinterpret_cast<const uint4*>(static_cast<const uint16_t*>(a.res2) + pix * a.res2_cstride +
                                                                         a.res_choff + slice * NOUT);
#pragma unroll
                        for (int i = 0; i < NOUT / 8; ++i) {
                            float f8[8];
                            unpack16x8(r2[i], a.res16_fmt, f8);
#pragma unroll
                            for (int e = 0; e < 8; ++e) val[8 * i + e] = __fadd_rn(__fmul_rn(val[8 * i + e], 0.2f), f8[e]);
                        }
                    } else {
                        const float4* r2 = reinterpret_cast<const float4*>(static_cast<const float*>(a.res2) + pix * a.res2_cstride +
                                                                           a.res_choff + slice * NOUT);
#pragma unroll
                        for (int i = 0; i < NOUT / 4; ++i) {
                            const float4 r4 = __ldg(r2 + i);
                            val[4 * i + 0] = __fadd_rn(__fmul_rn(val[4 * i + 0], 0.2f), r4.x);
                            val[4 * i + 1] = __fadd_rn(__fmul_rn(val[4 * i + 1], 0.2f), r4.y);
                            val[4 * i + 2] = __fadd_rn(__fmul_rn(val[4 * i + 2], 0.2f), r4.z);
                            val[4 * i + 3] = __fadd_rn(__fmul_rn(val[4 * i + 3], 0.2f), r4.w);
                        }
                    }
                }
                if (a.ep_mode == EP_ADD2 && a.res2) {
                    const size_t pix = (static_cast<size_t>(valid ? n : 0) * a.H + y) * a.W + (valid ? x : 0);
                    const float4* r2 = reinterpret_cast<const float4*>(static_cast<const float*>(a.res2) + pix * a.res2_cstride + a.res_choff + slice * NOUT);
#pragma unroll
                    for (int i = 0; i < NOUT / 4; ++i) {
                        const float4 r4 = __ldg(r2 + i);
                        val[4 * i + 0] = fmaf(a.res2_scale, r4.x, val[4 * i + 0]);
                        val[4 * i + 1] = fmaf(a.res2_scale, r4.y, val[4 * i + 1]);
                        val[4 * i + 2] = fmaf(a.res2_scale, r4.z, val[4 * i + 2]);
                        val[4 * i + 3] = fmaf(a.res2_scale, r4.w, val[4 * i + 3]);
                    }
                }
                if (a.lrelu) {
#pragma unroll
                    for (int i = 0; i < NOUT / 2; ++i) {
                        const float2 t = __fmul2_rn(make_float2(val[2 * i], val[2 * i + 1]), make_float2(0.2f, 0.2f));
                        val[2 * i] = fmaxf(val[2 * i], t.x);
                        val[2 * i + 1] = fmaxf(val[2 * i + 1], t.y);
                    }
                }
                if (a.out_nchw_raw && valid) {
                    const size_t plane = static_cast<size_t>(a.H) * a.W;
                    float* o = a.out_nchw_raw + static_cast<size_t>(n) * a.out_nchw_c * plane + static_cast<size_t>(y) * a.W + x;
#pragma unroll
                    for (int c = 0; c < NOUT; ++c) {
                        const int cc = slice * NOUT + c;
                        if (cc < a.out_nchw_c) o[static_cast<size_t>(cc) * plane] = val[c];
                    }
                }
                if (a.clamp01) {
#pragma unroll
                    for (int i = 0; i < NOUT; ++i) val[i] = fminf(fmaxf(val[i], 0.f), 1.f);
                }
                if (use_outf) {
#pragma unroll
                    for (int i = 0; i < NOUT / 4; ++i)
                        *reinterpret_cast<float4*>(tileR + m * 128 + ((i ^ (m & 7)) << 4)) =
                            make_float4(val[4 * i], val[4 * i + 1], val[4 * i + 2], val[4 * i + 3]);
                }
                if (use_o16 && a.mask16) {
                    const size_t pix = (static_cast<size_t>(valid ? n : 0) * a.H + y) * a.W + (valid ? x : 0);
                    const uint4* mk = reinterpret_cast<const uint4*>(static_cast<const uint16_t*>(a.mask16) + pix * a.mask16_cstride +
                                                                     a.mask16_choff + slice * NOUT);
#pragma unroll
                    for (int i = 0; i < NOUT / 8; ++i) {
                        const uint4 q4 = __ldg(mk + i);
                        const uint32_t w4[4] = {q4.x, q4.y, q4.z, q4.w};
#pragma unroll
                        for (int e = 0; e < 8; ++e) {
                            const uint32_t h16 = (w4[e >> 1] >> ((e & 1) * 16)) & 0xFFFFu;
                            const bool pos = ((h16 & 0x8000u) == 0) && ((h16 & 0x7FFFu) != 0);
                            if (!pos) val[8 * i + e] = __fmul_rn(val[8 * i + e], 0.2f);
                        }
                    }
                }
                if (use_o16 && a.out16_scale != 0.f) {
#pragma unroll
                    for (int i = 0; i < NOUT; ++i) val[i] = __fmul_rn(val[i], a.out16_scale);
                }
                if (use_o16) {
                    uint32_t pk[NOUT / 2];
#pragma unroll
                    for (int i = 0; i < NOUT / 2; ++i) {
                        if (a.out16_fmt == 1) {
                            __nv_bfloat162 h = __floats2bfloat162_rn(val[2 * i], val[2 * i + 1]);
                            pk[i] = *reinterpret_cast<uint32_t*>(&h);
                        } else {

                            pk[i] = pack_f16x2_sat(val[2 * i], val[2 * i + 1]);
                        }
                    }
                    uint4* dst = reinterpret_cast<uint4*>(tile16 + m * (NOUT * 2));
#pragma unroll
                    for (int i = 0; i < NOUT / 8; ++i) dst[i] = make_uint4(pk[4 * i], pk[4 * i + 1], pk[4 * i + 2], pk[4 * i + 3]);
                }
                if (staged) {
                    fence_proxy_async_smem();
                    named_bar_sync(1 + gi, 128);
                    if (lead_warp) {
                      if (elect_one()) {
                        if (use_outf && !DBGF(1) && !DBGF(64)) tma_store_4d(&tmapOF, tileR, a.outf_choff + slice * NOUT, x0, y, n0);
                        if (use_o16 && !DBGF(1) && !(DBGF(128) && a.has_res1)) {
                            const int c0 = a.out16_choff + (a.out16_slice_fixed ? 0 : slice * NOUT);
                            if (!a.out16_up2) {
                                tma_store_4d(&tmapO16, tile16, c0, x0, y, n0);
                            } else {
#pragma unroll
                                for (int s = 0; s < 4; ++s) tma_store_5d(&tmapO16, tile16, c0, s & 1, x0, 2 * y + (s >> 1), n0);
                            }
                        }
                        tma_store_commit();
                      }
                      __syncwarp();
                    }
                }
                if (a.out_nchw && valid) {
                    const size_t plane = static_cast<size_t>(a.H) * a.W;
                    float* o = a.out_nchw + static_cast<size_t>(n) * a.out_nchw_c * plane + static_cast<size_t>(y) * a.W + x;
#pragma unroll
                    for (int c = 0; c < NOUT; ++c) {
                        const int cc = slice * NOUT + c;
                        if (cc < a.out_nchw_c) o[static_cast<size_t>(cc) * plane] = val[c];
                    }
                }
                if (a.out_u8 && valid) {
                    unsigned char* o = a.out_u8 + ((static_cast<size_t>(n) * a.H + y) * a.W + x) * a.out_nchw_c;
#pragma unroll
                    for (int c = 0; c < NOUT; ++c) {
                        const int cc = slice * NOUT + c;
                        if (cc < a.out_nchw_c) o[cc] = static_cast<unsigned char>(fminf(fmaxf(__fmul_rn(val[c], 255.f), 0.f), 255.f));
                    }
                }
            }
            v0 += n_acc;
            g += yb - ya;
        }
        if (lead_warp) tma_store_wait_all();
        if (gi == 0 && lead_warp) RESR_DBG(6);
    }

    tc_fence_before();
    __syncthreads();
    if (threadIdx.x == 0) RESR_DBG(7);
    if (warp == 2) tmem_dealloc(tbase, 512);
}


bool conv3x3_plan_smem(ConvArgs* a, int cout_slice) {
    const int wbytes = a->nchunks * 3 * (3 * cout_slice) * 128;
    int nepi = a->has_outf ? 2 : 3;
    const char* env = getenv("RESR_CONV_NEPI");
    if (env) nepi = atoi(env);
    if (nepi < 1) nepi = 1;
    if (nepi > 3) nepi = 3;
    for (;; --nepi) {
        a->nepi = nepi;
        const int fixed = 1024 + wbytes + nepi * epi_group_bytes(*a, cout_slice) + kMiscBytes;
        int ns = (kSmemMax - fixed) / kStageBytes;
        if (ns > kMaxStages) ns = kMaxStages;
        if (ns >= 4 || nepi == 1) {
            a->nstages = ns;
            return ns >= 2;
        }
    }
}

void conv3x3_pick_tile(int W, int* BW, int* BN) {
    if (W == 64 || W == 32 || W == 16 || W == 8) {
        *BW = W;
        *BN = 128 / W;
    } else {
        *BW = 128;
        *BN = 1;
    }
}

typedef CUresult (*PFN_encodeTiled)(CUtensorMap*, CUtensorMapDataType, cuuint32_t, void*, const cuuint64_t*,
                                    const cuuint64_t*, const cuuint32_t*, const cuuint32_t*, CUtensorMapInterleave,
                                    CUtensorMapSwizzle, CUtensorMapL2promotion, CUtensorMapFloatOOBfill);

static PFN_encodeTiled get_encode_fn() {
    static PFN_encodeTiled fn = nullptr;
    if (!fn) {
        void* p = nullptr;
        cudaDriverEntryPointQueryResult q;
        if (cudaGetDriverEntryPoint("cuTensorMapEncodeTiled", &p, cudaEnableDefault, &q) == cudaSuccess &&
            q == cudaDriverEntryPointSuccess)
            fn = reinterpret_cast<PFN_encodeTiled>(p);
    }
    return fn;
}

int conv3x3_make_tmap_act(CUtensorMap* out, const void* base, int N, int H, int W, int C, int mode, int BW, int BN,
                          int cvalid) {
    PFN_encodeTiled enc = get_encode_fn();
    if (!enc) return -1;
    int cdim = cvalid > 0 ? (cvalid + 7) / 8 * 8 : C;
    if (cdim > C) cdim = C;
    const cuuint64_t dims[4] = {static_cast<cuuint64_t>(cdim), static_cast<cuuint64_t>(W), static_cast<cuuint64_t>(H),
                                static_cast<cuuint64_t>(N)};
    const cuuint64_t strides[3] = {static_cast<cuuint64_t>(C) * 2, static_cast<cuuint64_t>(W) * C * 2,
                                   static_cast<cuuint64_t>(H) * W * C * 2};
    cuuint32_t box[4] = {64, static_cast<cuuint32_t>(mode == 0 ? BW + 2 : BW), 1, static_cast<cuuint32_t>(mode == 0 ? 1 : BN)};
    const cuuint32_t estr[4] = {1, 1, 1, 1};
    static const int env_promo = getenv("RESR_TMAP_PROMO") ? atoi(getenv("RESR_TMAP_PROMO")) : -1;
    CUtensorMapL2promotion promo = (cdim % 64 != 0) ? CU_TENSOR_MAP_L2_PROMOTION_L2_64B : CU_TENSOR_MAP_L2_PROMOTION_L2_128B;
    if (env_promo == 0) promo = CU_TENSOR_MAP_L2_PROMOTION_NONE;
    else if (env_promo == 1) promo = CU_TENSOR_MAP_L2_PROMOTION_L2_64B;
    else if (env_promo == 2) promo = CU_TENSOR_MAP_L2_PROMOTION_L2_128B;
    else if (env_promo == 3) promo = CU_TENSOR_MAP_L2_PROMOTION_L2_256B;
    const CUresult r = enc(out, CU_TENSOR_MAP_DATA_TYPE_UINT16, 4, const_cast<void*>(base), dims, strides, box, estr,
                           CU_TENSOR_MAP_INTERLEAVE_NONE, CU_TENSOR_MAP_SWIZZLE_128B, promo, CU_TENSOR_MAP_FLOAT_OOB_FILL_NONE);
    return r == CUDA_SUCCESS ? 0 : static_cast<int>(r);
}

int conv3x3_make_tmap_out16(CUtensorMap* out, const void* base, int N, int H, int W, int C, int nout, int BW, int BN,
                            int up2) {
    PFN_encodeTiled enc = get_encode_fn();
    if (!enc) return -1;
    const cuuint32_t estr[5] = {1, 1, 1, 1, 1};
    CUresult r;
    if (!up2) {
        const cuuint64_t dims[4] = {static_cast<cuuint64_t>(C), static_cast<cuuint64_t>(W), static_cast<cuuint64_t>(H),
                                    static_cast<cuuint64_t>(N)};
        const cuuint64_t strides[3] = {static_cast<cuuint64_t>(C) * 2, static_cast<cuuint64_t>(W) * C * 2,
                                       static_cast<cuuint64_t>(H) * W * C * 2};
        const cuuint32_t box[4] = {static_cast<cuuint32_t>(nout), static_cast<cuuint32_t>(BW), 1, static_cast<cuuint32_t>(BN)};
        r = enc(out, CU_TENSOR_MAP_DATA_TYPE_UINT16, 4, const_cast<void*>(base), dims, strides, box, estr,
                CU_TENSOR_MAP_INTERLEAVE_NONE, CU_TENSOR_MAP_SWIZZLE_NONE, CU_TENSOR_MAP_L2_PROMOTION_NONE,
                CU_TENSOR_MAP_FLOAT_OOB_FILL_NONE);
    } else {
        const cuuint64_t dims[5] = {static_cast<cuuint64_t>(C), 2, static_cast<cuuint64_t>(W), static_cast<cuuint64_t>(2 * H),
                                    static_cast<cuuint64_t>(N)};
        const cuuint64_t strides[4] = {static_cast<cuuint64_t>(C) * 2, static_cast<cuuint64_t>(C) * 4,
                                       static_cast<cuuint64_t>(2 * W) * C * 2, static_cast<cuuint64_t>(2 * H) * 2 * W * C * 2};
        const cuuint32_t box[5] = {static_cast<cuuint32_t>(nout), 1, static_cast<cuuint32_t>(BW), 1, static_cast<cuuint32_t>(BN)};
        r = enc(out, CU_TENSOR_MAP_DATA_TYPE_UINT16, 5, const_cast<void*>(base), dims, strides, box, estr,
                CU_TENSOR_MAP_INTERLEAVE_NONE, CU_TENSOR_MAP_SWIZZLE_NONE, CU_TENSOR_MAP_L2_PROMOTION_NONE,
                CU_TENSOR_MAP_FLOAT_OOB_FILL_NONE);
    }
    return r == CUDA_SUCCESS ? 0 : static_cast<int>(r);
}

int conv3x3_make_tmap_f32(CUtensorMap* out, const void* base, int N, int H, int W, int C, int BW, int BN) {
    PFN_encodeTiled enc = get_encode_fn();
    if (!enc) return -1;
    const cuuint64_t dims[4] = {static_cast<cuuint64_t>(C), static_cast<cuuint64_t>(W), static_cast<cuuint64_t>(H),
                                static_cast<cuuint64_t>(N)};
    const cuuint64_t strides[3] = {static_cast<cuuint64_t>(C) * 4, static_cast<cuuint64_t>(W) * C * 4,
                                   static_cast<cuuint64_t>(H) * W * C * 4};
    const cuuint32_t box[4] = {32, static_cast<cuuint32_t>(BW), 1, static_cast<cuuint32_t>(BN)};
    const cuuint32_t estr[4] = {1, 1, 1, 1};
    const CUresult r = enc(out, CU_TENSOR_MAP_DATA_TYPE_FLOAT32, 4, const_cast<void*>(base), dims, strides, box, estr,
                           CU_TENSOR_MAP_INTERLEAVE_NONE, CU_TENSOR_MAP_SWIZZLE_128B, CU_TENSOR_MAP_L2_PROMOTION_L2_128B,
                           CU_TENSOR_MAP_FLOAT_OOB_FILL_NONE);
    return r == CUDA_SUCCESS ? 0 : static_cast<int>(r);
}

template <int NOUT>
static cudaError_t launch_t(const ConvMaps& maps, const ConvArgs& args, dim3 grid, int threads, cudaStream_t stream) {
    static PerDevice<bool> attr;
    if (!attr.cur()) {
        const cudaError_t e = cudaFuncSetAttribute(conv3x3_tc_kernel<NOUT>, cudaFuncAttributeMaxDynamicSharedMemorySize, kSmemMax);
        if (e != cudaSuccess) return e;
        attr.cur() = true;
    }
    cudaLaunchConfig_t cfg;
    memset(&cfg, 0, sizeof(cfg));
    cfg.gridDim = grid;
    cfg.blockDim = dim3(threads, 1, 1);
    cfg.dynamicSmemBytes = kSmemMax;
    cfg.stream = stream;
    cudaLaunchAttribute at[1];
    at[0].id = cudaLaunchAttributeProgrammaticStreamSerialization;
    at[0].val.programmaticStreamSerializationAllowed = 1;
    cfg.attrs = at;
    cfg.numAttrs = 1;
    return cudaLaunchKernelEx(&cfg, conv3x3_tc_kernel<NOUT>, maps.a, maps.o16, maps.of, args);
}

cudaError_t conv3x3_launch(const ConvMaps& maps, const ConvArgs& args, int cout_slice, int nslices, int num_sms,
                           cudaStream_t stream) {
    const int wbytes = args.nchunks * 3 * (3 * cout_slice) * 128;
    const int smem = 1024 + wbytes + args.nstages * kStageBytes + args.nepi * epi_group_bytes(args, cout_slice) + kMiscBytes;
    if (args.nstages < 2 || args.nepi < 1 || args.nepi > 3 || smem > kSmemMax) return cudaErrorInvalidConfiguration;
    long long gx = num_sms / nslices;
    const long long min_rows = 4;
    const long long cap = (args.rows_total + min_rows - 1) / min_rows;
    if (gx > cap) gx = cap;
    if (gx < 1) gx = 1;
    if (args.rows_total * (gx + 1) >= (1ll << 31)) return cudaErrorInvalidValue;
    const dim3 grid(static_cast<unsigned>(gx), static_cast<unsigned>(nslices), 1);
    const int threads = 128 + 128 * args.nepi;
    static const int env_flags = getenv("RESR_CONV_DBGFLAGS") ? atoi(getenv("RESR_CONV_DBGFLAGS")) : 0;
    if (env_flags && !(args.dbg_flags & 0x40000000)) {
        ConvArgs fixed = args;
        fixed.dbg_flags |= env_flags | 0x40000000;
        return conv3x3_launch(maps, fixed, cout_slice, nslices, num_sms, stream);
    }
    if (args.tail_ksteps != 1 && args.tail_ksteps != 2 && args.tail_ksteps != 4) {
        ConvArgs fixed = args;
        fixed.tail_ksteps = 4;
        return conv3x3_launch(maps, fixed, cout_slice, nslices, num_sms, stream);
    }
    if (cout_slice == 32) return launch_t<32>(maps, args, grid, threads, stream);
    if (cout_slice == 16) return launch_t<16>(maps, args, grid, threads, stream);
    return cudaErrorInvalidValue;
}

}
```

real_esrgan-pytorch_b200/csrc/gen_internal.cuh:

```cuda
#pragma once
#include <cstddef>
#include <cstdint>
#include <vector>

#include "conv3x3.cuh"

namespace resr {

struct ConvSpec {
    int cin, cout;
    int nout;
    int nslices;
    int nchunks;
    int fmt;
    size_t p_off;
    size_t w_off;
    size_t b_off;
    size_t wt_off;
    int t_nslices;
    int t_nchunks;
};

static const int kNumConvs = 351;
static const int kNumRRDB = 23;

struct Table {
    ConvSpec c[kNumConvs];
    size_t n_params, pack_bytes, bias_floats, packt_bytes;
    Table() {
        int i = 0;
        auto add = [&](int cin, int cout, int fmt) {
            ConvSpec& s = c[i++];
            s.cin = cin;
            s.cout = cout;
            s.nout = cout >= 32 ? 32 : 16;
            s.nslices = (cout + s.nout - 1) / s.nout;
            s.nchunks = (cin + 63) / 64;
            s.fmt = fmt;
        };
        add(3, 64, 0);
        for (int r = 0; r < kNumRRDB * 3; ++r) {
            for (int k = 0; k < 4; ++k) add(64 + 32 * k, 32, 0);
            add(192, 64, 0);
        }
        add(64, 64, 0);
        add(64, 64, 0);
        add(64, 64, 0);
        add(64, 64, 0);
        add(64, 3, 0);
        size_t p = 0, w = 0, b = 0, wt = 0;
        for (int k = 0; k < kNumConvs; ++k) {
            c[k].p_off = p;
            p += static_cast<size_t>(c[k].cout) * c[k].cin * 9 + c[k].cout;
            c[k].w_off = w;
            w += static_cast<size_t>(c[k].nslices) * c[k].nchunks * 3 * (3 * c[k].nout) * 128;
            c[k].b_off = b;
            b += static_cast<size_t>(c[k].nslices) * c[k].nout;
            c[k].t_nslices = (c[k].cin + 31) / 32;
            c[k].t_nchunks = (c[k].cout + 63) / 64;
            c[k].wt_off = wt;
            wt += static_cast<size_t>(c[k].t_nslices) * c[k].t_nchunks * 3 * 96 * 128;
        }
        n_params = p;
        pack_bytes = w;
        bias_floats = b;
        packt_bytes = wt;
    }
};
inline const Table& table() {
    static Table t;
    return t;
}


struct Step {
    int conv;
    ConvMaps maps;
    ConvArgs a;
    ConvLaunchCfg cfg;
};

struct Plan {
    int N = 0, H = 0, W = 0;
    void* ws = nullptr;
    std::vector<Step> steps;
    uint16_t* xin = nullptr;
    int pair_policy = -1;
    bool valid = false;
};

}

struct resr_generator {
    cudaGraphExec_t step_exec = nullptr;
    const void* step_key[6] = {nullptr, nullptr, nullptr, nullptr, nullptr, nullptr};
    int step_shape[3] = {0, 0, 0};
    bool step_graph_failed = false;
    cudaStream_t h2d_stream = nullptr, d2h_stream = nullptr;
    cudaEvent_t ev_h2d[2] = {nullptr, nullptr}, ev_fwd[2] = {nullptr, nullptr}, ev_d2h[2] = {nullptr, nullptr};
    unsigned long long host_calls = 0;
    int host_shape[3] = {0, 0, 0};
    const void* host_ws = nullptr;
    cudaStream_t side_stream = nullptr;
    cudaEvent_t ev_fork = nullptr, ev_dy = nullptr, ev_join = nullptr;
    cudaEvent_t ev_dyc[3] = {nullptr, nullptr, nullptr};
    bool ev_dyc_valid[3] = {false, false, false};
    cudaEvent_t ev_bucket[4] = {nullptr, nullptr, nullptr, nullptr};
    uint8_t* wpack_t = nullptr;
    uint8_t* wpack_t2 = nullptr;
    float* zero_bias = nullptr;
    bool packed_t = false;
    const float* flat_params = nullptr;
    uint8_t* wpack = nullptr;
    void* pack_jobs = nullptr;
    void* pack_jobs_t = nullptr;
    float* bias = nullptr;
    bool loaded = false;
    int num_sms = 148;
    int force_mode = -1;
    int precision = 0;
    resr::Plan plan;
};


namespace resr {
int grid_for(size_t total, int block);
void ensure_transposed_packs(resr_generator* g, cudaStream_t s, bool force);
int launch_pack_all(resr_generator* g, const float* flat, int transposed, cudaStream_t s);
int launch_pack_rdb_bwd(resr_generator* g, const float* flat, uint8_t* wpack_t2, cudaStream_t s);
void launch_pack_conv(const float* w, const float* bias, uint16_t* wp, float* bp, int cin, int cout, int nout, int nslices,
                      int nchunks, int fmt, int transposed, cudaStream_t s);
}
```

real_esrgan-pytorch_b200/csrc/generator.cu:

```cuda
#include <cuda_bf16.h>
#include <cuda_fp16.h>

#include <cstdio>
#include <cstdlib>
#include <cstring>
#include <vector>

#include "../../include/resr.h"
#include "conv3x3.cuh"
#include "errors.h"
#include "gen_internal.cuh"

namespace resr {


__device__ __forceinline__ void pack_conv_body(const float* __restrict__ w, const float* __restrict__ bias, uint16_t* __restrict__ wp,
                                               float* __restrict__ bp, int cin, int cout, int nout, int nslices, int nchunks, int fmt,
                                               int transposed, size_t first, size_t stride) {
    const int NT = 3 * nout;
    const size_t total = static_cast<size_t>(nslices) * nchunks * 3 * NT * 64;
    for (size_t idx = first; idx < total; idx += stride) {
        const int k = static_cast<int>(idx & 63);
        unsigned t = static_cast<unsigned>(idx >> 6);
        const int n = t % NT;
        t /= NT;
        const int dx = t % 3;
        t /= 3;
        const int chunk = t % nchunks;
        const int slice = static_cast<int>(t / nchunks);
        const int co = slice * nout + n % nout;
        const int dy = n / nout;
        const int ci = chunk * 64 + k;
        float v = 0.f;
        if (!transposed) {
            if (co < cout && ci < cin) v = w[((static_cast<size_t>(co) * cin + ci) * 3 + dy) * 3 + dx];
        } else {
            if (co < cin && ci < cout) v = w[((static_cast<size_t>(ci) * cin + co) * 3 + (2 - dy)) * 3 + (2 - dx)];
        }
        uint16_t bits;
        if (fmt == 1) {
            __nv_bfloat16 h = __float2bfloat16_rn(v);
            bits = *reinterpret_cast<uint16_t*>(&h);
        } else {
            __half h = __float2half_rn(v);
            bits = *reinterpret_cast<uint16_t*>(&h);
        }
        const size_t tile = ((static_cast<size_t>(slice) * nchunks + chunk) * 3 + dx) * NT * 64;
        const size_t off = tile + static_cast<size_t>(n) * 64 + ((((k >> 3) ^ (n & 7)) << 3) | (k & 7));
        wp[off] = bits;
    }
    const int nb = nslices * nout;
    if (bp)
        for (size_t i = first; i < static_cast<size_t>(nb); i += stride) bp[i] = (i < static_cast<size_t>(cout) && bias) ? bias[i] : 0.f;
}

__global__ void pack_conv_kernel(const float* __restrict__ w, const float* __restrict__ bias, uint16_t* __restrict__ wp,
                                 float* __restrict__ bp, int cin, int cout, int nout, int nslices, int nchunks, int fmt,
                                 int transposed) {
    pack_conv_body(w, bias, wp, bp, cin, cout, nout, nslices, nchunks, fmt, transposed,
                   blockIdx.x * static_cast<size_t>(blockDim.x) + threadIdx.x, static_cast<size_t>(gridDim.x) * blockDim.x);
}

struct PackJob {
    unsigned long long p_off, w_off, b_off;
    int cin, cout, nout, nslices, nchunks, fmt;
};
__global__ void __launch_bounds__(256) pack_all_kernel(const float* __restrict__ flat, const PackJob* __restrict__ jobs,
                                                       uint8_t* __restrict__ wpack, float* __restrict__ bias, int transposed) {
    const PackJob j = jobs[blockIdx.y];
    const float* w = flat + j.p_off;
    const float* b = w + static_cast<size_t>(j.cout) * j.cin * 9;
    pack_conv_body(w, transposed ? nullptr : b, reinterpret_cast<uint16_t*>(wpack + j.w_off), transposed ? nullptr : bias + j.b_off,
                   j.cin, j.cout, j.nout, j.nslices, j.nchunks, j.fmt, transposed,
                   blockIdx.x * static_cast<size_t>(blockDim.x) + threadIdx.x, static_cast<size_t>(gridDim.x) * blockDim.x);
}

__global__ void __launch_bounds__(256) pack_rdb_bwd_kernel(const float* __restrict__ flat, const PackJob* __restrict__ jobs,
                                                          uint8_t* __restrict__ wpack) {
    const int r = blockIdx.z, b = 4 - static_cast<int>(blockIdx.y);
    const PackJob shape = jobs[1 + 5 * r + blockIdx.y];
    const int cin_p = 64 + 32 * (4 - b);
    const int cout_p = b == 0 ? 64 : 32;
    const int NT = 3 * shape.nout;
    uint16_t* wp = reinterpret_cast<uint16_t*>(wpack + shape.w_off);
    const size_t total = static_cast<size_t>(shape.nslices) * shape.nchunks * 3 * NT * 64;
    for (size_t idx = blockIdx.x * static_cast<size_t>(blockDim.x) + threadIdx.x; idx < total;
         idx += static_cast<size_t>(gridDim.x) * blockDim.x) {
        const int k = static_cast<int>(idx & 63);
        unsigned t = static_cast<unsigned>(idx >> 6);
        const int n = t % NT;
        t /= NT;
        const int dx = t % 3;
        t /= 3;
        const int chunk = t % shape.nchunks;
        const int slice = static_cast<int>(t / shape.nchunks);
        const int co = slice * shape.nout + n % shape.nout;
        const int dy = n / shape.nout;
        const int ci = chunk * 64 + k;
        float v = 0.f;
        if (co < cout_p && ci < cin_p) {
            const int l = ci < 64 ? 5 : 4 - (ci - 64) / 32;
            const int co_l = ci < 64 ? ci : (ci - 64) % 32;
            const int cin_l = 64 + 32 * (l - 1);
            const int cin_idx = b == 0 ? co : 64 + 32 * (b - 1) + co;
            const PackJob lay = jobs[1 + 5 * r + (l - 1)];
            v = flat[lay.p_off + ((static_cast<size_t>(co_l) * cin_l + cin_idx) * 3 + (2 - dy)) * 3 + (2 - dx)];
        }
        const __nv_bfloat16 h = __float2bfloat16_rn(v);
        const size_t tile = ((static_cast<size_t>(slice) * shape.nchunks + chunk) * 3 + dx) * NT * 64;
        wp[tile + static_cast<size_t>(n) * 64 + ((((k >> 3) ^ (n & 7)) << 3) | (k & 7))] = *reinterpret_cast<const uint16_t*>(&h);
    }
}

__global__ void nchw_to_nhwc16_kernel(const float* __restrict__ x, uint16_t* __restrict__ out, int N, int C, int H, int W,
                                      int c_pad, int fmt) {
    const size_t npix = static_cast<size_t>(N) * H * W;
    const int groups = c_pad / 8;
    const size_t total = npix * groups;
    const size_t plane = static_cast<size_t>(H) * W;
    for (size_t idx = blockIdx.x * static_cast<size_t>(blockDim.x) + threadIdx.x; idx < total;
         idx += static_cast<size_t>(gridDim.x) * blockDim.x) {
        const int gch = idx % groups;
        const size_t pix = idx / groups;
        const size_t n = pix / plane, rem = pix % plane;
        uint32_t pk[4];
#pragma unroll
        for (int j = 0; j < 4; ++j) {
            float v[2];
#pragma unroll
            for (int e = 0; e < 2; ++e) {
                const int c = gch * 8 + 2 * j + e;
                v[e] = c < C ? x[(n * C + c) * plane + rem] : 0.f;
            }
            if (fmt == 1) {
                __nv_bfloat162 h = __floats2bfloat162_rn(v[0], v[1]);
                pk[j] = *reinterpret_cast<uint32_t*>(&h);
            } else {
                __half2 h = __floats2half2_rn(v[0], v[1]);
                pk[j] = *reinterpret_cast<uint32_t*>(&h);
            }
        }
        reinterpret_cast<uint4*>(out + pix * c_pad)[gch] = make_uint4(pk[0], pk[1], pk[2], pk[3]);
    }
}

__global__ void u8nhwc_to_nhwc16_kernel(const unsigned char* __restrict__ x, uint16_t* __restrict__ out, size_t npix, int C, int c_pad,
                                        int fmt) {
    const int groups = c_pad / 8;
    const size_t total = npix * groups;
    for (size_t idx = blockIdx.x * static_cast<size_t>(blockDim.x) + threadIdx.x; idx < total;
         idx += static_cast<size_t>(gridDim.x) * blockDim.x) {
        const int gch = idx % groups;
        const size_t pix = idx / groups;
        uint32_t pk[4];
#pragma unroll
        for (int j = 0; j < 4; ++j) {
            float v[2];
#pragma unroll
            for (int e = 0; e < 2; ++e) {
                const int c = gch * 8 + 2 * j + e;
                v[e] = c < C ? __fdiv_rn(static_cast<float>(x[pix * C + c]), 255.f) : 0.f;
            }
            if (fmt == 1) {
                __nv_bfloat162 h = __floats2bfloat162_rn(v[0], v[1]);
                pk[j] = *reinterpret_cast<uint32_t*>(&h);
            } else {
                __half2 h = __floats2half2_rn(v[0], v[1]);
                pk[j] = *reinterpret_cast<uint32_t*>(&h);
            }
        }
        reinterpret_cast<uint4*>(out + pix * c_pad)[gch] = make_uint4(pk[0], pk[1], pk[2], pk[3]);
    }
}

__global__ void tensor_to_image_kernel(const float* __restrict__ x, unsigned char* __restrict__ out, int C, size_t HW, int range_norm,
                                       int half) {
    const size_t total = HW * C;
    for (size_t idx = blockIdx.x * static_cast<size_t>(blockDim.x) + threadIdx.x; idx < total;
         idx += static_cast<size_t>(gridDim.x) * blockDim.x) {
        const int c = idx % C;
        const size_t p = idx / C;
        float v = x[static_cast<size_t>(c) * HW + p];
        if (range_norm) v = __fdiv_rn(__fadd_rn(v, 1.f), 2.f);
        if (half) {
            const __half h = __hmul(__float2half_rn(v), __float2half_rn(255.f));
            v = fminf(fmaxf(__half2float(h), 0.f), 255.f);
        } else {
            v = fminf(fmaxf(__fmul_rn(v, 255.f), 0.f), 255.f);
        }
        out[idx] = static_cast<unsigned char>(v);
    }
}

int grid_for(size_t total, int block) {
    size_t g = (total + block - 1) / block;
    if (g > 148 * 16) g = 148 * 16;
    if (g < 1) g = 1;
    return static_cast<int>(g);
}

int launch_pack_all(resr_generator* g, const float* flat, int transposed, cudaStream_t s) {
    const Table& T = table();
    PackJob** slot = reinterpret_cast<PackJob**>(transposed ? &g->pack_jobs_t : &g->pack_jobs);
    if (!*slot) {
        std::vector<PackJob> h(kNumConvs);
        for (int k = 0; k < kNumConvs; ++k) {
            const ConvSpec& c = T.c[k];
            PackJob& j = h[k];
            j.p_off = c.p_off;
            j.cin = c.cin; j.cout = c.cout;
            if (!transposed) {
                j.w_off = c.w_off; j.b_off = c.b_off; j.nout = c.nout; j.nslices = c.nslices; j.nchunks = c.nchunks;
                j.fmt = g->precision == 1 ? 1 : c.fmt;
            } else {
                j.w_off = c.wt_off; j.b_off = 0; j.nout = 32; j.nslices = c.t_nslices; j.nchunks = c.t_nchunks; j.fmt = 1;
            }
        }
        if (cudaMalloc(slot, kNumConvs * sizeof(PackJob)) != cudaSuccess) return -1;
        cudaMemcpyAsync(*slot, h.data(), kNumConvs * sizeof(PackJob), cudaMemcpyHostToDevice, s);
        cudaStreamSynchronize(s);
    }
    const int first = transposed ? 1 : 0;
    pack_all_kernel<<<dim3(24, kNumConvs - first), 256, 0, s>>>(flat, *slot + first, transposed ? g->wpack_t : g->wpack, g->bias,
                                                                transposed);
    return cudaGetLastError() == cudaSuccess ? 0 : -2;
}

int launch_pack_rdb_bwd(resr_generator* g, const float* flat, uint8_t* wpack_t2, cudaStream_t s) {
    if (!g->pack_jobs) return -1;
    pack_rdb_bwd_kernel<<<dim3(8, 5, kNumRRDB * 3), 256, 0, s>>>(flat, static_cast<const PackJob*>(g->pack_jobs), wpack_t2);
    return cudaGetLastError() == cudaSuccess ? 0 : -2;
}

void launch_pack_conv(const float* w, const float* bias, uint16_t* wp, float* bp, int cin, int cout, int nout, int nslices,
                      int nchunks, int fmt, int transposed, cudaStream_t s) {
    const size_t total = static_cast<size_t>(nslices) * nchunks * 3 * (3 * nout) * 64;
    pack_conv_kernel<<<grid_for(total, 256), 256, 0, s>>>(w, bias, wp, bp, cin, cout, nout, nslices, nchunks, fmt, transposed);
}

static size_t align_up(size_t v, size_t a) { return (v + a - 1) / a * a; }

struct WsLayout {
    size_t xin, c[3], f0, m[4], t1, t2, t3, t4, total;
};
static WsLayout ws_layout(size_t N, size_t H, size_t W, int precision = 0) {
    const size_t P = N * H * W;
    WsLayout L;
    size_t o = 0;
    auto take = [&](size_t bytes) {
        const size_t at = o;
        o = align_up(o + bytes, 1024);
        return at;
    };
    L.xin = take(P * 64 * 2);
    for (int i = 0; i < 3; ++i) L.c[i] = take(P * 192 * 2);
    L.f0 = take(P * 64 * 4);
    for (int i = 0; i < 4; ++i) L.m[i] = precision == 1 ? take(P * 64 * 4) : 0;
    L.t1 = take(4 * P * 64 * 2);
    L.t2 = take(16 * P * 64 * 2);
    L.t3 = take(16 * P * 64 * 2);
    L.t4 = take(16 * P * 64 * 2);
    L.total = o;
    return L;
}

static int build_plan(resr_generator* g, int N, int H, int W, void* ws, cudaStream_t s) {
    Plan& p = g->plan;
    p.valid = false;
    p.steps.clear();
    p.N = N; p.H = H; p.W = W; p.ws = ws;
    p.pair_policy = conv3x3_set_pair_policy(-1);
    const int prec = g->precision;
    const WsLayout L = ws_layout(N, H, W, prec);
    uint8_t* base = static_cast<uint8_t*>(ws);
    uint16_t* xin = reinterpret_cast<uint16_t*>(base + L.xin);
    uint16_t* cbuf[3];
    for (int i = 0; i < 3; ++i) cbuf[i] = reinterpret_cast<uint16_t*>(base + L.c[i]);
    float* F0 = reinterpret_cast<float*>(base + L.f0);
    float* M[4];
    for (int i = 0; i < 4; ++i) M[i] = reinterpret_cast<float*>(base + L.m[i]);
    uint16_t* t1 = reinterpret_cast<uint16_t*>(base + L.t1);
    uint16_t* t2 = reinterpret_cast<uint16_t*>(base + L.t2);
    uint16_t* t3 = reinterpret_cast<uint16_t*>(base + L.t3);
    uint16_t* t4 = reinterpret_cast<uint16_t*>(base + L.t4);
    p.xin = xin;

    struct Geo { int H, W, BW, BN, mode; };
    Geo geo[3];
    for (int s = 0; s < 3; ++s) {
        geo[s].H = H << s;
        geo[s].W = W << s;
        conv3x3_pick_tile(geo[s].W, &geo[s].BW, &geo[s].BN);
        geo[s].mode = geo[s].BN == 1 ? 0 : 1;
        if (g->force_mode >= 0) geo[s].mode = (geo[s].BN == 1) ? g->force_mode : 1;
    }
    for (int i = 0; i < 3; ++i) cudaMemsetAsync(cbuf[i], 0, static_cast<size_t>(N) * H * W * 192 * 2, s);

    const Table& T = table();
    int map_rc = 0;
    auto make_step = [&](int conv, int s, const void* in16, int cin_total) {
        const ConvSpec& cs = T.c[conv];
        const Geo& q = geo[s];
        Step st;
        memset(&st, 0, sizeof(st));
        st.conv = conv;
        ConvArgs& a = st.a;
        a.N = N; a.H = q.H; a.W = q.W; a.BW = q.BW; a.BN = q.BN;
        a.nxs = (q.W + q.BW - 1) / q.BW;
        a.ncg = ((N + q.BN - 1) / q.BN) * a.nxs;
        a.nchunks = cs.nchunks;
        a.tail_ksteps = conv3x3_tail_ksteps(cs.cin);
        a.mode = q.mode;
        a.fmt_in = prec == 1 ? 1 : cs.fmt;
        a.rows_total = static_cast<long long>(a.ncg) * q.H;
        a.wpack = g->wpack + cs.w_off;
        a.bias = g->bias + cs.b_off;
        map_rc |= conv3x3_make_tmap_act(&st.maps.a, in16, N, q.H, q.W, cin_total, q.mode, q.BW, q.BN, cs.cin);
        return st;
    };
    auto set_out16 = [&](Step& st, int s, void* dst, int c_total, int choff, int fmt, int up2) {
        const Geo& q = geo[s];
        st.a.has_out16 = 1; st.a.out16_fmt = prec == 1 ? 1 : fmt; st.a.out16_choff = choff; st.a.out16_up2 = up2;
        map_rc |= conv3x3_make_tmap_out16(&st.maps.o16, dst, N, q.H, q.W, c_total, T.c[st.conv].nout, q.BW, q.BN, up2);
    };
    auto set_outf = [&](Step& st, float* dst) {
        st.a.has_outf = 1; st.a.outf_choff = 0; st.a.outf = static_cast<float*>(dst); st.a.outf_cstride = 64;
        map_rc |= conv3x3_make_tmap_f32(&st.maps.of, dst, N, geo[0].H, geo[0].W, 64, geo[0].BW, geo[0].BN);
    };
    auto set_res1 = [&](Step& st, const float* src) {
        st.a.has_res1 = 1; st.a.res_choff = 0; st.a.res1 = src; st.a.res1_cstride = 64;
    };
    auto push = [&](Step& st) {
        if (!conv3x3_choose(&st.a, T.c[st.conv].nout, T.c[st.conv].nslices, &st.cfg)) map_rc |= 1 << 20;
        static const int serp = getenv("RESR_CONV_SERPENTINE") ? atoi(getenv("RESR_CONV_SERPENTINE")) : 1;
        st.a.reverse = (serp && st.cfg.pair) ? static_cast<int>(p.steps.size() & 1) : 0;
        p.steps.push_back(st);
    };

    auto set_res16 = [&](Step& st, const uint16_t* src) {
        st.a.has_res1 = 1; st.a.res_choff = 0; st.a.res1 = src; st.a.res1_cstride = 192;
        st.a.res16 = 1; st.a.res16_fmt = 0;
    };
    int conv = 0;
    {
        Step st = make_step(conv, 0, xin, 64);
        st.a.ep_mode = EP_PLAIN;
        set_outf(st, F0);
        set_out16(st, 0, cbuf[0], 192, 0, 0, 0);
        push(st);
        ++conv;
    }
    for (int i = 0; i < kNumRRDB; ++i) {
        for (int j = 0; j < 3; ++j) {
            uint16_t* cin_buf = cbuf[j];
            for (int k = 0; k < 4; ++k) {
                Step st = make_step(conv, 0, cin_buf, 192);
                st.a.ep_mode = EP_PLAIN; st.a.lrelu = 1;
                set_out16(st, 0, cin_buf, 192, 64 + 32 * k, 0, 0);
                push(st);
                ++conv;
            }
            Step st = make_step(conv, 0, cin_buf, 192);
            st.a.ep_mode = j < 2 ? EP_RDB : EP_RRDB;
            if (prec == 1) {
                const int t = i * 3 + j;
                set_res1(st, t == 0 ? F0 : M[t % 4]);
                if (j == 2) { st.a.res2 = i == 0 ? F0 : M[(3 * i) % 4]; st.a.res2_cstride = 64; }
                set_outf(st, M[(t + 1) % 4]);
            } else {
                set_res16(st, cin_buf);
                if (j == 2) { st.a.res2 = cbuf[0]; st.a.res2_cstride = 192; }
            }
            set_out16(st, 0, cbuf[(j + 1) % 3], 192, 0, 0, 0);
            push(st);
            ++conv;
        }
    }
    {
        Step st = make_step(conv, 0, cbuf[0], 192);
        st.a.ep_mode = EP_SKIP;
        set_res1(st, F0);
        set_out16(st, 0, t1, 64, 0, 0, 1);
        push(st);
        ++conv;
    }
    {
        Step st = make_step(conv, 1, t1, 64);
        st.a.lrelu = 1;
        set_out16(st, 1, t2, 64, 0, 0, 1);
        push(st);
        ++conv;
    }
    {
        Step st = make_step(conv, 2, t2, 64);
        st.a.lrelu = 1;
        set_out16(st, 2, t3, 64, 0, 0, 0);
        push(st);
        ++conv;
    }
    {
        Step st = make_step(conv, 2, t3, 64);
        st.a.lrelu = 1;
        set_out16(st, 2, t4, 64, 0, 0, 0);
        push(st);
        ++conv;
    }
    {
        Step st = make_step(conv, 2, t4, 64);
        st.a.clamp01 = 1;
        st.a.out_nchw = nullptr; st.a.out_nchw_c = 3;
        push(st);
        ++conv;
    }
    if (map_rc != 0) return set_error(RESR_E_CUDA, "tensor map / shared memory planning failed (%d)", map_rc);
    if (cudaGetLastError() != cudaSuccess) return set_error(RESR_E_CUDA, "workspace init failed");
    p.valid = true;
    return RESR_OK;
}

}

using namespace resr;

extern "C" {

int resr_version(void) { return 1; }

size_t resr_generator_num_params(void) { return table().n_params; }
int resr_generator_num_tensors(void) { return 2 * kNumConvs; }
int resr_generator_launches_per_forward(void) { return 1 + kNumConvs; }

int resr_set_conv_pair_policy(int policy) { return conv3x3_set_pair_policy(policy); }

int resr_debug_wait_profile(unsigned long long* out16_host, int reset) {
    if (conv3x3_wait_profile(out16_host, reset) != 0) return set_error(RESR_E_CUDA, "wait profile copy failed");
    return RESR_OK;
}

int resr_generator_tensor_span(int index, size_t* offset, size_t* count) {
    if (index < 0 || index >= 2 * kNumConvs || !offset || !count) return set_error(RESR_E_INVALID, "bad tensor index");
    const ConvSpec& c = table().c[index / 2];
    const size_t wn = static_cast<size_t>(c.cout) * c.cin * 9;
    if (index % 2 == 0) { *offset = c.p_off; *count = wn; }
    else { *offset = c.p_off + wn; *count = c.cout; }
    return RESR_OK;
}

int resr_generator_create(resr_generator_t** out, int in_channels, int out_channels, int upscale_factor) {
    if (!out) return set_error(RESR_E_INVALID, "null out");
    if (in_channels != 3 || out_channels != 3 || upscale_factor != 4)
        return set_error(RESR_E_INVALID, "only Generator(3, 3, 4) is implemented (got %d, %d, %d)", in_channels,
                         out_channels, upscale_factor);
    int dev = 0;
    if (cudaGetDevice(&dev) != cudaSuccess) return set_error(RESR_E_CUDA, "no CUDA device: %s", cudaGetErrorString(cudaGetLastError()));
    cudaDeviceProp prop;
    if (cudaGetDeviceProperties(&prop, dev) != cudaSuccess) return set_error(RESR_E_CUDA, "cudaGetDeviceProperties failed");
    if (prop.major != 10) return set_error(RESR_E_CUDA, "libresr needs an sm_100a device (found sm_%d%d)", prop.major, prop.minor);
    resr_generator* g = new resr_generator();
    g->num_sms = prop.multiProcessorCount;
    if (getenv("RESR_NUM_SMS") && atoi(getenv("RESR_NUM_SMS")) > 0 && atoi(getenv("RESR_NUM_SMS")) < g->num_sms)
        g->num_sms = atoi(getenv("RESR_NUM_SMS"));
    const char* fm = getenv("RESR_CONV_MODE");
    if (fm) g->force_mode = atoi(fm);
    if (cudaMalloc(&g->wpack, table().pack_bytes) != cudaSuccess || cudaMalloc(&g->bias, table().bias_floats * 4) != cudaSuccess) {
        delete g;
        return set_error(RESR_E_CUDA, "cudaMalloc of packed weights failed");
    }
    *out = g;
    return RESR_OK;
}

void resr_generator_destroy(resr_generator_t* g) {
    if (!g) return;
    cudaFree(g->wpack);
    cudaFree(g->bias);
    cudaFree(g->wpack_t);
    cudaFree(g->wpack_t2);
    cudaFree(g->pack_jobs);
    cudaFree(g->pack_jobs_t);
    cudaFree(g->zero_bias);
    if (g->step_exec) cudaGraphExecDestroy(g->step_exec);
    if (g->h2d_stream) cudaStreamDestroy(g->h2d_stream);
    if (g->d2h_stream) cudaStreamDestroy(g->d2h_stream);
    for (int i = 0; i < 2; ++i) {
        if (g->ev_h2d[i]) cudaEventDestroy(g->ev_h2d[i]);
        if (g->ev_fwd[i]) cudaEventDestroy(g->ev_fwd[i]);
        if (g->ev_d2h[i]) cudaEventDestroy(g->ev_d2h[i]);
    }
    if (g->side_stream) cudaStreamDestroy(g->side_stream);
    if (g->ev_fork) cudaEventDestroy(g->ev_fork);
    if (g->ev_dy) cudaEventDestroy(g->ev_dy);
    if (g->ev_join) cudaEventDestroy(g->ev_join);
    for (int i = 0; i < 3; ++i)
        if (g->ev_dyc[i]) cudaEventDestroy(g->ev_dyc[i]);
    for (int i = 0; i < 4; ++i)
        if (g->ev_bucket[i]) cudaEventDestroy(g->ev_bucket[i]);
    delete g;
}

int resr_generator_load_params(resr_generator_t* g, const float* flat, void* stream) {
    if (!g || !flat) return set_error(RESR_E_INVALID, "null argument");
    cudaStream_t s = static_cast<cudaStream_t>(stream);
    const Table& T = table();
    if (launch_pack_all(g, flat, 0, s) != 0) return set_error(RESR_E_CUDA, "weight packing failed");
    const cudaError_t e = cudaGetLastError();
    if (e != cudaSuccess) return set_error(RESR_E_CUDA, "pack kernels: %s", cudaGetErrorString(e));
    g->loaded = true;
    g->packed_t = false;
    g->flat_params = flat;
    ensure_transposed_packs(g, s, false);
    return RESR_OK;
}

size_t resr_generator_workspace_bytes(int n, int h, int w) {
    if (n <= 0 || h <= 0 || w <= 0) return 0;
    return ws_layout(n, h, w).total;
}

size_t resr_generator_workspace_bytes_for(const resr_generator_t* g, int n, int h, int w) {
    if (!g || n <= 0 || h <= 0 || w <= 0) return 0;
    return ws_layout(n, h, w, g->precision).total;
}

int resr_generator_set_precision(resr_generator_t* g, int precision) {
    if (!g) return set_error(RESR_E_INVALID, "null argument");
    if (precision != 0 && precision != 1) return set_error(RESR_E_INVALID, "precision must be 0 (fp16) or 1 (bf16 + fp32 residual masters)");
    if (g->precision != precision) {
        g->precision = precision;
        g->loaded = false;
        g->plan.valid = false;
        cudaFree(g->pack_jobs);
        g->pack_jobs = nullptr;
    }
    return RESR_OK;
}

static int forward_any(resr_generator_t* g, const float* x, const unsigned char* x_u8, float* y, unsigned char* y_u8, int n, int h, int w,
                       void* workspace, size_t workspace_bytes, void* stream);

int resr_generator_forward(resr_generator_t* g, const float* x, float* y, int n, int h, int w, void* workspace,
                           size_t workspace_bytes, void* stream) {
    if (!x || !y) return set_error(RESR_E_INVALID, "null argument");
    return forward_any(g, x, nullptr, y, nullptr, n, h, w, workspace, workspace_bytes, stream);
}

int resr_generator_forward_u8(resr_generator_t* g, const unsigned char* x_u8, unsigned char* y_u8, int n, int h, int w, void* workspace,
                              size_t workspace_bytes, void* stream) {
    if (!x_u8 || !y_u8) return set_error(RESR_E_INVALID, "null argument");
    return forward_any(g, nullptr, x_u8, nullptr, y_u8, n, h, w, workspace, workspace_bytes, stream);
}

int resr_generator_forward_u8_host(resr_generator_t* g, const unsigned char* x_host, unsigned char* y_host, int n, int h, int w,
                                   void* workspace, size_t workspace_bytes, void* stream) {
    if (!g || !x_host || !y_host) return set_error(RESR_E_INVALID, "null argument");
    cudaStream_t s = static_cast<cudaStream_t>(stream);
    const size_t in_bytes = static_cast<size_t>(n) * 3 * h * w, out_bytes = in_bytes * 16;
    const size_t need = resr_generator_workspace_bytes_for(g, n, h, w);
    const size_t off_x = (need + 1023) / 1024 * 1024, off_y = off_x + (in_bytes + 1023) / 1024 * 1024;
    if (workspace_bytes < off_y + out_bytes) return set_error(RESR_E_NOMEM, "workspace too small for u8 host staging (need %zu)", off_y + out_bytes);
    unsigned char* xd = static_cast<unsigned char*>(workspace) + off_x;
    unsigned char* yd = static_cast<unsigned char*>(workspace) + off_y;
    if (cudaMemcpyAsync(xd, x_host, in_bytes, cudaMemcpyHostToDevice, s) != cudaSuccess) return set_error(RESR_E_CUDA, "H2D failed");
    const int rc = resr_generator_forward_u8(g, xd, yd, n, h, w, workspace, need, stream);
    if (rc != RESR_OK) return rc;
    if (cudaMemcpyAsync(y_host, yd, out_bytes, cudaMemcpyDeviceToHost, s) != cudaSuccess) return set_error(RESR_E_CUDA, "D2H failed");
    const cudaError_t e = cudaStreamSynchronize(s);
    if (e != cudaSuccess) return set_error(RESR_E_CUDA, "forward_u8_host: %s", cudaGetErrorString(e));
    return RESR_OK;
}

int resr_tensor_to_image_u8(const float* x, unsigned char* out_hwc, int c, int h, int w, int range_norm, int half, void* stream) {
    if (!x || !out_hwc || c <= 0 || h <= 0 || w <= 0) return set_error(RESR_E_INVALID, "bad argument");
    const size_t HW = static_cast<size_t>(h) * w;
    tensor_to_image_kernel<<<grid_for(HW * c, 256), 256, 0, static_cast<cudaStream_t>(stream)>>>(x, out_hwc, c, HW, range_norm, half);
    const cudaError_t e = cudaGetLastError();
    if (e != cudaSuccess) return set_error(RESR_E_CUDA, "tensor_to_image: %s", cudaGetErrorString(e));
    return RESR_OK;
}

static int forward_any(resr_generator_t* g, const float* x, const unsigned char* x_u8, float* y, unsigned char* y_u8, int n, int h, int w,
                       void* workspace, size_t workspace_bytes, void* stream) {
    if (!g || !workspace) return set_error(RESR_E_INVALID, "null argument");
    if (n <= 0 || h <= 0 || w <= 0) return set_error(RESR_E_INVALID, "bad shape %dx3x%dx%d", n, h, w);
    if (!g->loaded) return set_error(RESR_E_INVALID, "resr_generator_load_params has not been called");
    if (workspace_bytes < resr_generator_workspace_bytes_for(g, n, h, w)) return set_error(RESR_E_NOMEM, "workspace too small");
    if ((reinterpret_cast<uintptr_t>(workspace) & 1023) != 0) return set_error(RESR_E_INVALID, "workspace must be 1024-byte aligned");
    cudaStream_t s = static_cast<cudaStream_t>(stream);
    Plan& p = g->plan;
    if (!p.valid || p.N != n || p.H != h || p.W != w || p.ws != workspace || p.pair_policy != conv3x3_set_pair_policy(-1)) {
        const int rc = build_plan(g, n, h, w, workspace, s);
        if (rc != RESR_OK) return rc;
    }
    const size_t total = static_cast<size_t>(n) * h * w * 8;
    if (x_u8) u8nhwc_to_nhwc16_kernel<<<grid_for(total, 256), 256, 0, s>>>(x_u8, p.xin, static_cast<size_t>(n) * h * w, 3, 64, g->precision == 1 ? 1 : 0);
    else nchw_to_nhwc16_kernel<<<grid_for(total, 256), 256, 0, s>>>(x, p.xin, n, 3, h, w, 64, g->precision == 1 ? 1 : 0);
    const Table& T = table();
    for (size_t i = 0; i < p.steps.size(); ++i) {
        Step& st = p.steps[i];
        if (i + 1 == p.steps.size()) { st.a.out_nchw = y; st.a.out_u8 = y_u8; }
        const cudaError_t e = conv3x3_run(st.maps, st.a, st.cfg, g->num_sms, s);
        if (e != cudaSuccess) return set_error(RESR_E_CUDA, "conv %d launch: %s", st.conv, cudaGetErrorString(e));
    }
    return RESR_OK;
}

int resr_generator_forward_host(resr_generator_t* g, const float* x_host, float* y_host, int n, int h, int w,
                                void* workspace, size_t workspace_bytes, void* stream) {
    if (!x_host || !y_host) return set_error(RESR_E_INVALID, "null argument");
    cudaStream_t s = static_cast<cudaStream_t>(stream);
    const size_t in_bytes = static_cast<size_t>(n) * 3 * h * w * 4, out_bytes = in_bytes * 16;
    const size_t need = resr_generator_workspace_bytes_for(g, n, h, w);
    const size_t off_x = (need + 1023) / 1024 * 1024, off_y = off_x + (in_bytes + 1023) / 1024 * 1024;
    if (workspace_bytes < off_y + out_bytes) return set_error(RESR_E_NOMEM, "workspace too small for host staging (need %zu)", off_y + out_bytes);
    float* xd = reinterpret_cast<float*>(static_cast<uint8_t*>(workspace) + off_x);
    float* yd = reinterpret_cast<float*>(static_cast<uint8_t*>(workspace) + off_y);
    if (cudaMemcpyAsync(xd, x_host, in_bytes, cudaMemcpyHostToDevice, s) != cudaSuccess) return set_error(RESR_E_CUDA, "H2D failed");
    const int rc = resr_generator_forward(g, xd, yd, n, h, w, workspace, need, stream);
    if (rc != RESR_OK) return rc;
    if (cudaMemcpyAsync(y_host, yd, out_bytes, cudaMemcpyDeviceToHost, s) != cudaSuccess) return set_error(RESR_E_CUDA, "D2H failed");
    const cudaError_t e = cudaStreamSynchronize(s);
    if (e != cudaSuccess) return set_error(RESR_E_CUDA, "forward_host: %s", cudaGetErrorString(e));
    return RESR_OK;
}

int resr_generator_forward_host_async(resr_generator_t* g, const float* x_host, float* y_host, int n, int h, int w,
                                      void* workspace, size_t workspace_bytes, void* stream) {
    if (!g || !x_host || !y_host) return set_error(RESR_E_INVALID, "null argument");
    cudaStream_t s = static_cast<cudaStream_t>(stream);
    const size_t in_bytes = static_cast<size_t>(n) * 3 * h * w * 4, out_bytes = in_bytes * 16;
    const size_t need = resr_generator_workspace_bytes_for(g, n, h, w);
    const size_t in_al = (in_bytes + 1023) / 1024 * 1024, out_al = (out_bytes + 1023) / 1024 * 1024;
    const size_t off0 = (need + 1023) / 1024 * 1024;
    if (workspace_bytes < off0 + 2 * (in_al + out_al))
        return set_error(RESR_E_NOMEM, "workspace too small for two host staging slots (need %zu)", off0 + 2 * (in_al + out_al));
    if (!g->h2d_stream) {
        if (cudaStreamCreateWithFlags(&g->h2d_stream, cudaStreamNonBlocking) != cudaSuccess ||
            cudaStreamCreateWithFlags(&g->d2h_stream, cudaStreamNonBlocking) != cudaSuccess)
            return set_error(RESR_E_CUDA, "cannot create copy streams");
        for (int i = 0; i < 2; ++i) {
            cudaEventCreateWithFlags(&g->ev_h2d[i], cudaEventDisableTiming);
            cudaEventCreateWithFlags(&g->ev_fwd[i], cudaEventDisableTiming);
            cudaEventCreateWithFlags(&g->ev_d2h[i], cudaEventDisableTiming);
        }
    }
    if (g->host_calls > 0 && (g->host_shape[0] != n || g->host_shape[1] != h || g->host_shape[2] != w || g->host_ws != workspace)) {
        cudaStreamSynchronize(g->h2d_stream);
        cudaStreamSynchronize(s);
        cudaStreamSynchronize(g->d2h_stream);
        g->host_calls = 0;
    }
    g->host_shape[0] = n; g->host_shape[1] = h; g->host_shape[2] = w; g->host_ws = workspace;
    const int slot = static_cast<int>(g->host_calls & 1);
    const bool reused = g->host_calls >= 2;
    uint8_t* base = static_cast<uint8_t*>(workspace) + off0 + static_cast<size_t>(slot) * (in_al + out_al);
    float* xd = reinterpret_cast<float*>(base);
    float* yd = reinterpret_cast<float*>(base + in_al);
    if (reused) cudaStreamWaitEvent(g->h2d_stream, g->ev_fwd[slot], 0);
    if (cudaMemcpyAsync(xd, x_host, in_bytes, cudaMemcpyHostToDevice, g->h2d_stream) != cudaSuccess) return set_error(RESR_E_CUDA, "H2D failed");
    cudaEventRecord(g->ev_h2d[slot], g->h2d_stream);
    cudaStreamWaitEvent(s, g->ev_h2d[slot], 0);
    if (reused) cudaStreamWaitEvent(s, g->ev_d2h[slot], 0);
    const int rc = resr_generator_forward(g, xd, yd, n, h, w, workspace, need, stream);
    if (rc != RESR_OK) return rc;
    cudaEventRecord(g->ev_fwd[slot], s);
    cudaStreamWaitEvent(g->d2h_stream, g->ev_fwd[slot], 0);
    if (cudaMemcpyAsync(y_host, yd, out_bytes, cudaMemcpyDeviceToHost, g->d2h_stream) != cudaSuccess) return set_error(RESR_E_CUDA, "D2H failed");
    cudaEventRecord(g->ev_d2h[slot], g->d2h_stream);
    ++g->host_calls;
    return RESR_OK;
}

int resr_generator_host_sync(resr_generator_t* g) {
    if (!g) return set_error(RESR_E_INVALID, "null argument");
    if (!g->d2h_stream) return RESR_OK;
    cudaError_t e = cudaStreamSynchronize(g->h2d_stream);
    if (e == cudaSuccess) e = cudaStreamSynchronize(g->d2h_stream);
    if (e != cudaSuccess) return set_error(RESR_E_CUDA, "host_sync: %s", cudaGetErrorString(e));
    return RESR_OK;
}

int resr_nchw_to_nhwc16(const float* x, void* out16, int n, int c, int h, int w, int c_pad, int fmt, void* stream) {
    if (!x || !out16 || c_pad % 8 != 0 || c > c_pad) return set_error(RESR_E_INVALID, "bad argument");
    const size_t total = static_cast<size_t>(n) * h * w * (c_pad / 8);
    nchw_to_nhwc16_kernel<<<grid_for(total, 256), 256, 0, static_cast<cudaStream_t>(stream)>>>(
        x, static_cast<uint16_t*>(out16), n, c, h, w, c_pad, fmt);
    const cudaError_t e = cudaGetLastError();
    if (e != cudaSuccess) return set_error(RESR_E_CUDA, "nchw_to_nhwc16: %s", cudaGetErrorString(e));
    return RESR_OK;
}

int resr_conv3x3(const resr_conv_desc* d, void* stream) {
    if (!d || !d->in16 || !d->weight) return set_error(RESR_E_INVALID, "null argument");
    if (d->cin > d->c_total || d->c_total % 8 != 0) return set_error(RESR_E_INVALID, "bad channel counts");
    cudaStream_t s = static_cast<cudaStream_t>(stream);
    int dev = 0, sms = 148;
    cudaGetDevice(&dev);
    cudaDeviceGetAttribute(&sms, cudaDevAttrMultiProcessorCount, dev);
    const int nout = d->cout >= 32 ? 32 : 16;
    const int nslices = (d->cout + nout - 1) / nout;
    const int nchunks = (d->cin + 63) / 64;
    if (nchunks * 64 > d->c_total) return set_error(RESR_E_INVALID, "c_total must cover cin rounded up to 64");
    const size_t pack_bytes = static_cast<size_t>(nslices) * nchunks * 3 * (3 * nout) * 128;
    uint8_t* wp = nullptr;
    float* bp = nullptr;
    if (cudaMalloc(&wp, pack_bytes) != cudaSuccess || cudaMalloc(&bp, nslices * nout * 4) != cudaSuccess)
        return set_error(RESR_E_CUDA, "cudaMalloc failed");
    launch_pack_conv(d->weight, d->bias, reinterpret_cast<uint16_t*>(wp), bp, d->cin, d->cout, nout, nslices, nchunks,
                     d->fmt_in, 0, s);
    cudaStreamSynchronize(s);
    ConvArgs a;
    ConvMaps maps;
    memset(&a, 0, sizeof(a));
    memset(&maps, 0, sizeof(maps));
    a.N = d->n; a.H = d->h; a.W = d->w;
    conv3x3_pick_tile(d->w, &a.BW, &a.BN);
    a.mode = d->mode >= 0 ? d->mode : (a.BN == 1 ? 0 : 1);
    if (a.BN != 1) a.mode = 1;
    a.nxs = (d->w + a.BW - 1) / a.BW;
    a.ncg = ((d->n + a.BN - 1) / a.BN) * a.nxs;
    a.nchunks = nchunks;
    a.tail_ksteps = conv3x3_tail_ksteps(d->cin);
    a.fmt_in = d->fmt_in;
    a.rows_total = static_cast<long long>(a.ncg) * d->h;
    a.wpack = wp; a.bias = bp;
    a.ep_mode = d->ep_mode; a.lrelu = d->lrelu; a.clamp01 = d->clamp01;
    int rc = conv3x3_make_tmap_act(&maps.a, d->in16, d->n, d->h, d->w, d->c_total, a.mode, a.BW, a.BN, d->cin);
    if (d->out16) {
        a.has_out16 = 1; a.out16_fmt = d->out16_fmt; a.out16_choff = d->out16_choff; a.out16_up2 = d->out16_up2;
        rc |= conv3x3_make_tmap_out16(&maps.o16, d->out16, d->n, d->h, d->w, d->out16_cstride, nout, a.BW, a.BN, d->out16_up2);
    }
    if (d->outf) {
        a.has_outf = 1; a.outf_choff = d->outf_choff; a.outf = static_cast<float*>(d->outf); a.outf_cstride = d->outf_cstride;
        rc |= conv3x3_make_tmap_f32(&maps.of, d->outf, d->n, d->h, d->w, d->outf_cstride, a.BW, a.BN);
    }
    if (d->res1) {
        a.has_res1 = 1; a.res_choff = d->res_choff; a.res1 = d->res1; a.res1_cstride = d->res_cstride;
        a.res16 = d->res16; a.res16_fmt = d->res16_fmt;
    }
    a.res2 = d->res2; a.res2_cstride = d->res_cstride;
    a.out_nchw = d->out_nchw; a.out_nchw_c = d->out_nchw_c;
    a.dbg = d->dbg;
    a.dbg_flags = d->dbg_flags;
    ConvLaunchCfg cfg;
    if (!conv3x3_choose(&a, nout, nslices, &cfg)) rc |= 1 << 20;
    if (nout == 16 && (d->out16 || d->outf || d->res1)) rc |= 1 << 21;
    cudaError_t e = cudaSuccess;
    if (rc == 0) e = conv3x3_run(maps, a, cfg, sms, s);
    const cudaError_t e2 = cudaStreamSynchronize(s);
    cudaFree(wp);
    cudaFree(bp);
    if (rc != 0) return set_error(RESR_E_CUDA, "tensor map / shared memory planning failed (%d)", rc);
    if (e != cudaSuccess) return set_error(RESR_E_CUDA, "conv launch: %s", cudaGetErrorString(e));
    if (e2 != cudaSuccess) return set_error(RESR_E_CUDA, "conv run: %s", cudaGetErrorString(e2));
    return RESR_OK;
}

}
```

Before: 24.62.

## Fold nearest-2x upsample into following 3x3 conv via phase-decomposed 2x2 weights

Adds an in_up2 path that runs each upsampling conv on the low-resolution input. The weights are pre-summed into per-phase 2x2 taps (fold packing), so the nearest-neighbour upsampled tensor never has to be materialized. Each output-column phase runs as a separate grid slice and produces two output rows per input row. This cuts the MAC count per output by about 4/9 and halves input traffic, at the cost of more complex accumulator ring bookkeeping and extra packed weights.

```diff
diff --git a/include/resr.h b/include/resr.h
--- a/include/resr.h
+++ b/include/resr.h
@@ -72,6 +72,7 @@
     int out_nchw_c;
     int dbg_flags;
     unsigned long long* dbg;
+    int in_up2;
 } resr_conv_desc;
 int resr_conv3x3(const resr_conv_desc* d, void* stream);
 
diff --git a/real_esrgan-pytorch_b200/_lib.py b/real_esrgan-pytorch_b200/_lib.py
--- a/real_esrgan-pytorch_b200/_lib.py
+++ b/real_esrgan-pytorch_b200/_lib.py
@@ -28,6 +28,7 @@
         ("out_nchw_c", c_int),
         ("dbg_flags", c_int),
         ("dbg", c_void_p),
+        ("in_up2", c_int),
     ]
 
 
diff --git a/real_esrgan-pytorch_b200/csrc/conv3x3.cuh b/real_esrgan-pytorch_b200/csrc/conv3x3.cuh
--- a/real_esrgan-pytorch_b200/csrc/conv3x3.cuh
+++ b/real_esrgan-pytorch_b200/csrc/conv3x3.cuh
@@ -35,6 +35,7 @@
     int out16_fmt;
     int out16_choff;
     int out16_up2;
+    int in_up2;
     int has_outf;
     int outf_choff;
     float* outf;
diff --git a/real_esrgan-pytorch_b200/csrc/conv3x3_pair.cu b/real_esrgan-pytorch_b200/csrc/conv3x3_pair.cu
--- a/real_esrgan-pytorch_b200/csrc/conv3x3_pair.cu
+++ b/real_esrgan-pytorch_b200/csrc/conv3x3_pair.cu
@@ -67,9 +67,9 @@
     }
 }
 
-template <int NOUT, int KS, int I0, int I1>
+template <int NT, int KS, int I0, int I1>
 __device__ __forceinline__ void issue_range(uint32_t d0, uint32_t a_lo, uint32_t b_lo, uint32_t idesc) {
-    constexpr uint32_t WT = (3 * NOUT / 2 * 128) >> 4;
+    constexpr uint32_t WT = (NT / 2 * 128) >> 4;
 #pragma unroll
     for (int i = I0; i < I1; ++i) {
         const int dx = i / KS, ks = i % KS;
@@ -77,27 +77,41 @@
     }
 }
 
-template <int NOUT, int NDX, int HALF>
+template <int NT, int NDX, int HALF>
 __device__ __forceinline__ void issue_half(int ks, uint32_t d0, uint32_t a_lo, uint32_t b_lo, uint32_t idesc) {
 #define RESR_HALF(KS)                                                                       \
-    if (HALF == 0) issue_range<NOUT, KS, 0, (NDX * KS) / 2>(d0, a_lo, b_lo, idesc);          \
-    else issue_range<NOUT, KS, (NDX * KS) / 2, NDX * KS>(d0, a_lo, b_lo, idesc)
+    if (HALF == 0) issue_range<NT, KS, 0, (NDX * KS) / 2>(d0, a_lo, b_lo, idesc);            \
+    else issue_range<NT, KS, (NDX * KS) / 2, NDX * KS>(d0, a_lo, b_lo, idesc)
     if (ks == 2) { RESR_HALF(2); }
     else if (ks == 1) { RESR_HALF(1); }
     else { RESR_HALF(4); }
 #undef RESR_HALF
 }
 
-template <int NOUT, int MODE, int S>
+template <bool FOLD>
+struct StripAcc {
+    int pad, n_acc;
+    uint32_t vfirst;
+    __device__ __forceinline__ StripAcc(uint32_t v0, int ra, int rb) {
+        pad = FOLD ? static_cast<int>((v0 + 1) & 1u) : 0;
+        n_acc = FOLD ? pad + 2 * (rb - ra) + 4 : rb - ra + 3;
+        vfirst = v0 + pad + (FOLD ? 3 : 2);
+    }
+};
+
+template <int NOUT, bool FOLD, int MODE, int S>
 __device__ __forceinline__ void mma_role(const ConvArgs& a, const RowRange rr, const uint32_t tbase, const uint32_t wsm_addr,
                                          const uint32_t stg_addr, const uint32_t full_a, const uint32_t empty_a,
                                          const uint32_t accfull_a, const uint32_t slotfree_a) {
-    constexpr uint32_t WT = (3 * NOUT / 2 * 128) >> 4;
-    const uint32_t idesc = make_idesc_f16(a.fmt_in, 256, 3 * NOUT);
+    constexpr int NT = (FOLD ? 4 : 3) * NOUT;
+    constexpr int NTAP = FOLD ? 2 : 3;
+    constexpr uint32_t VSTEP = FOLD ? 2 : 1;
+    constexpr uint32_t WT = (NT / 2 * 128) >> 4;
+    const uint32_t idesc = make_idesc_f16(a.fmt_in, 256, NT);
     const uint32_t w_lo = (wsm_addr & 0x3FFFFu) >> 4;
-    const uint32_t s_lo = (stg_addr & 0x3FFFFu) >> 4;
-    const int nsteps = MODE == 0 ? a.nchunks : a.nchunks * 3;
-    const uint32_t b_step = (MODE == 0 ? 3 : 1) * WT;
+    const uint32_t s_lo = ((stg_addr & 0x3FFFFu) >> 4) + (FOLD && MODE == 0 ? blockIdx.y * 8u : 0u);
+    const int nsteps = MODE == 0 ? a.nchunks : a.nchunks * NTAP;
+    const uint32_t b_step = (MODE == 0 ? NTAP : 1) * WT;
     const int nstages = a.nstages;
     const int H = a.H;
     int stage = 0;
@@ -105,7 +119,7 @@
     uint32_t a_lo = s_lo;
     int pending_empty = -1;
     bool full_ready = false, slot_ready = false;
-    uint32_t vnew = 1;
+    uint32_t v0 = 0;
     uint32_t acq = 0;
     PROF_DECL(p_full); PROF_DECL(p_slot); PROF_DECL(p_steps);
     PROF_T0(p_t0);
@@ -113,22 +127,19 @@
         const int ya = g % H;
         const int yb = min(H, ya + (rr.g1 - g));
         const int ra = max(ya - 1, 0), rb = min(yb, H - 1);
-        vnew += 1;
-        for (int r = ra; r <= rb; ++r, ++vnew) {
-            if (slot_ready && acq == vnew) {
+        const StripAcc<FOLD> sa(v0, ra, rb);
+        uint32_t vnew = sa.vfirst;
+        for (int r = ra; r <= rb; ++r, vnew += VSTEP) {
+            if (slot_ready) ++acq;
+            PROF_T0(p_t);
+            while (static_cast<int>(vnew - acq) >= 0) {
+                mbar_wait_a(slotfree_a + (ring_slot<S>(acq) << 3), ring_parity<S>(acq));
                 ++acq;
-            } else {
-                PROF_T0(p_t);
-                while (static_cast<int>(vnew - acq) >= 0) {
-                    mbar_wait_a(slotfree_a + (ring_slot<S>(acq) << 3), ring_parity<S>(acq));
-                    ++acq;
-                }
-                PROF_ADD(p_slot, p_t);
             }
+            PROF_ADD(p_slot, p_t);
             slot_ready = false;
             tc_fence_after();
-            const uint32_t s0 = ring_slot<S>(vnew), s1 = ring_slot<S>(vnew - 1), s2 = ring_slot<S>(vnew - 2);
-            const uint32_t d0 = tbase + s0 * NOUT;
+            const uint32_t d0 = tbase + ring_slot<S>(vnew) * NOUT;
             uint32_t b_lo = w_lo;
             for (int st = 0; st < nsteps; ++st, b_lo += b_step) {
                 if (!full_ready) { PROF_T0(p_t); mbar_wait_a(full_a + (stage << 3), phase); PROF_ADD(p_full, p_t); }
@@ -137,9 +148,9 @@
                 ++p_steps;
 #endif
                 const bool last = (st == nsteps - 1);
-                const int ks = (st >= nsteps - (MODE == 0 ? 1 : 3)) ? a.tail_ksteps : 4;
+                const int ks = (st >= nsteps - (MODE == 0 ? 1 : NTAP)) ? a.tail_ksteps : 4;
                 if (elect_one()) {
-                    issue_half<NOUT, MODE == 0 ? 3 : 1, 0>(ks, d0, a_lo, b_lo, idesc);
+                    issue_half<NT, MODE == 0 ? NTAP : 1, 0>(ks, d0, a_lo, b_lo, idesc);
                     if (pending_empty >= 0) umma2_commit_mc(empty_a + (pending_empty << 3), 3);
                 }
                 __syncwarp();
@@ -147,21 +158,23 @@
                 const uint32_t a_cur = a_lo;
                 if (++stage == nstages) { stage = 0; phase ^= 1u; a_lo = s_lo; } else { a_lo += kStageBytes >> 4; }
                 full_ready = mbar_test_wait_a(full_a + (stage << 3), phase);
-                if (last && r < rb) slot_ready = mbar_test_wait_a(slotfree_a + (ring_slot<S>(vnew + 1) << 3), ring_parity<S>(vnew + 1));
+                if (last && r < rb) slot_ready = mbar_test_wait_a(slotfree_a + (ring_slot<S>(acq) << 3), ring_parity<S>(acq));
                 if (elect_one()) {
-                    issue_half<NOUT, MODE == 0 ? 3 : 1, 1>(ks, d0, a_cur, b_lo, idesc);
+                    issue_half<NT, MODE == 0 ? NTAP : 1, 1>(ks, d0, a_cur, b_lo, idesc);
                     if (last) {
-                        umma2_commit_mc(accfull_a + (s2 << 3), 3);
+                        if (FOLD) umma2_commit_mc(accfull_a + (ring_slot<S>(vnew - 3) << 3), 3);
+                        umma2_commit_mc(accfull_a + (ring_slot<S>(vnew - 2) << 3), 3);
+                        if (FOLD && r == ra && sa.pad) umma2_commit_mc(accfull_a + (ring_slot<S>(vnew - 4) << 3), 3);
                         if (r == rb) {
-                            umma2_commit_mc(accfull_a + (s1 << 3), 3);
-                            umma2_commit_mc(accfull_a + (s0 << 3), 3);
+                            umma2_commit_mc(accfull_a + (ring_slot<S>(vnew - 1) << 3), 3);
+                            umma2_commit_mc(accfull_a + (ring_slot<S>(vnew) << 3), 3);
                         }
                     }
                 }
                 __syncwarp();
             }
         }
-        vnew += 1;
+        v0 += sa.n_acc;
         g += yb - ya;
     }
     if (pending_empty >= 0) {
@@ -194,26 +207,34 @@
 
 }
 
-template <int NOUT>
+__host__ __device__ inline int pair_wbytes(const ConvArgs& a, int nout) {
+    return a.nchunks * (a.in_up2 ? 2 * (4 * nout / 2) : 3 * (3 * nout / 2)) * 128;
+}
+
+template <int NOUT, bool FOLD>
 __global__ void __launch_bounds__(512, 1)
 conv3x3_pair_kernel(const __grid_constant__ CUtensorMap tmapA, const __grid_constant__ CUtensorMap tmapO16,
                     const __grid_constant__ CUtensorMap tmapOF, const ConvArgs a) {
-    constexpr int NT = 3 * NOUT;
+    constexpr int NT = (FOLD ? 4 : 3) * NOUT;
     constexpr int NH = NT / 2;
     constexpr int WHALF = NH * 128;
+    constexpr int NTAP = FOLD ? 2 : 3;
     constexpr int NSUB = NOUT == 64 ? 2 : 1;
     constexpr int SUBW = NOUT / NSUB;
     constexpr int SLOTS = NOUT == 64 ? 8 : 16;
     constexpr int S = SLOTS - 2;
+    constexpr int TILE16W = FOLD ? NOUT : SUBW;
+    static_assert(!FOLD || NOUT == 64, "the folded geometry runs 64-channel pairs");
     extern __shared__ uint8_t smem_raw[];
     uint8_t* smem = smem_raw + ((1024u - (smem_u32(smem_raw) & 1023u)) & 1023u);
 
     const int warp = __shfl_sync(0xffffffffu, threadIdx.x >> 5, 0);
     const int lane = threadIdx.x & 31;
-    const int slice = blockIdx.y;
+    const int slice = FOLD ? 0 : blockIdx.y;
+    const int phb = FOLD ? static_cast<int>(blockIdx.y) : 0;
     const uint32_t rank = cluster_ctarank();
-    const uint32_t wbytes = static_cast<uint32_t>(a.nchunks) * 3u * WHALF;
-    const int epi_bytes = epi_group_bytes_pair(a, SUBW);
+    const uint32_t wbytes = static_cast<uint32_t>(a.nchunks) * NTAP * WHALF;
+    const int epi_bytes = epi_group_bytes_pair(a, TILE16W);
 
     uint8_t* wsm = smem;
     uint8_t* stg = smem + wbytes;
@@ -267,25 +288,39 @@
     if (warp == 0) {
         if (elect_one()) {
             mbar_expect_tx(wbar, wbytes);
-            constexpr int G = NOUT == 64 ? 32 : NOUT / 2;
-            constexpr int BPD = NOUT / G;
-            constexpr int NB = 3 * BPD / 2;
-            for (int c = 0; c < a.nchunks; ++c) {
-                for (int dx = 0; dx < 3; ++dx) {
-                    uint8_t* dst = wsm + (c * 3 + dx) * WHALF;
-#pragma unroll
-                    for (int j = 0; j < NB; ++j) {
-                        const int blk = static_cast<int>(rank) * NB + j;
-                        const int dyv = blk / BPD, part = blk % BPD;
-                        const int dy = a.reverse ? 2 - dyv : dyv;
-                        const uint8_t* src;
-                        if (NOUT == 64)
-                            src = a.wpack + ((static_cast<size_t>(slice * 2 + part) * a.nchunks + c) * 3 + dx) * (96 * 128) +
-                                  static_cast<size_t>(dy) * 32 * 128;
-                        else
-                            src = a.wpack + ((static_cast<size_t>(slice) * a.nchunks + c) * 3 + dx) * (NT * 128) +
-                                  static_cast<size_t>(dy * NOUT + part * G) * 128;
-                        bulk_load_1d(dst + j * G * 128, src, G * 128, wbar);
+            if (FOLD) {
+                for (int c = 0; c < a.nchunks; ++c) {
+                    for (int t = 0; t < 2; ++t) {
+                        const uint8_t* tile = a.wpack + ((static_cast<size_t>(phb) * a.nchunks + c) * 2 + t) * (NT * 128);
+#pragma unroll
+                        for (int j = 0; j < 2; ++j) {
+                            const int fv = 2 * static_cast<int>(rank) + j;
+                            const int f = a.reverse ? 3 - fv : fv;
+                            bulk_load_1d(wsm + (c * 2 + t) * WHALF + j * NOUT * 128, tile + f * NOUT * 128, NOUT * 128, wbar);
+                        }
+                    }
+                }
+            } else {
+                constexpr int G = NOUT == 64 ? 32 : NOUT / 2;
+                constexpr int BPD = NOUT / G;
+                constexpr int NB = 3 * BPD / 2;
+                for (int c = 0; c < a.nchunks; ++c) {
+                    for (int dx = 0; dx < 3; ++dx) {
+                        uint8_t* dst = wsm + (c * 3 + dx) * WHALF;
+#pragma unroll
+                        for (int j = 0; j < NB; ++j) {
+                            const int blk = static_cast<int>(rank) * NB + j;
+                            const int dyv = blk / BPD, part = blk % BPD;
+                            const int dy = a.reverse ? 2 - dyv : dyv;
+                            const uint8_t* src;
+                            if (NOUT == 64)
+                                src = a.wpack + ((static_cast<size_t>(slice * 2 + part) * a.nchunks + c) * 3 + dx) * (96 * 128) +
+                                      static_cast<size_t>(dy) * 32 * 128;
+                            else
+                                src = a.wpack + ((static_cast<size_t>(slice) * a.nchunks + c) * 3 + dx) * (NT * 128) +
+                                      static_cast<size_t>(dy * NOUT + part * G) * 128;
+                            bulk_load_1d(dst + j * G * 128, src, G * 128, wbar);
+                        }
                     }
                 }
             }
@@ -294,7 +329,8 @@
         grid_dep_wait();
         int stage = 0;
         uint32_t phase = 0;
-        const int ndx = a.mode == 0 ? 1 : 3;
+        const int ndx = a.mode == 0 ? 1 : NTAP;
+        const int dx0 = a.mode == 0 ? 0 : phb;
         const uint32_t tx_bytes = a.mode == 0 ? (a.BW + 2) * 128 : 128 * 128;
         const uint32_t full0 = map_to_cta(smem_u32(full), 0);
         PROF_DECL(p_empty);
@@ -315,7 +351,7 @@
                         if (elect_one()) {
                             if (rank == 0) mbar_expect_tx(full + stage, 2 * tx_bytes);
                             tma_load_4d_pair(stg + stage * kStageBytes, &tmapA, full0 + (stage << 3), c * 64,
-                                             a.mode == 0 ? x0 - 1 : x0 + dx - 1, a.reverse ? H - 1 - r : r, n0);
+                                             a.mode == 0 ? x0 - 1 : x0 + dx0 + dx - 1, a.reverse ? H - 1 - r : r, n0);
                         }
                         __syncwarp();
                         if (++stage == a.nstages) { stage = 0; phase ^= 1; }
@@ -334,8 +370,8 @@
         if (rank == 0) {
             mbar_wait(wpair, 0);
             tc_fence_after();
-            if (a.mode == 0) mma_role<NOUT, 0, S>(a, rr, tbase, smem_u32(wsm), smem_u32(stg), smem_u32(full), smem_u32(empty), smem_u32(acc_full), smem_u32(slot_free));
-            else mma_role<NOUT, 1, S>(a, rr, tbase, smem_u32(wsm), smem_u32(stg), smem_u32(full), smem_u32(empty), smem_u32(acc_full), smem_u32(slot_free));
+            if (a.mode == 0) mma_role<NOUT, FOLD, 0, S>(a, rr, tbase, smem_u32(wsm), smem_u32(stg), smem_u32(full), smem_u32(empty), smem_u32(acc_full), smem_u32(slot_free));
+            else mma_role<NOUT, FOLD, 1, S>(a, rr, tbase, smem_u32(wsm), smem_u32(stg), smem_u32(full), smem_u32(empty), smem_u32(acc_full), smem_u32(slot_free));
         }
     } else if (warp >= 4) {
         const int gi = (warp - 4) >> 2;
@@ -343,7 +379,7 @@
         const int m = q * 32 + lane;
         const bool lead_warp = ((warp - 4) & 3) == 0;
         uint8_t* const tile_base = epi + gi * epi_bytes;
-        const int buf_bytes = epi_buf_bytes_pair(a, SUBW);
+        const int buf_bytes = epi_buf_bytes_pair(a, TILE16W);
         const bool two_bufs = a.epi_bufs == 2;
         uint32_t pass = 0;
         const uint32_t lane_base = tbase + (static_cast<uint32_t>(q * 32) << 16);
@@ -381,19 +417,22 @@
             const int x = x0 + x_in_tile;
             const bool valid = (n < a.N) && (x < a.W);
             const int ra = max(ya - 1, 0), rb = min(yb, H - 1);
-            const int n_acc = rb - ra + 3;
-            for (int j = 0; j < n_acc; ++j) {
+            const StripAcc<FOLD> sa(v0, ra, rb);
+            for (int j = 0; j < sa.n_acc; ++j) {
                 const uint32_t v = v0 + j;
                 if (static_cast<int>(v % a.nepi) != gi) continue;
-                const int yv = ra - 1 + j;
-                const bool emit = (yv >= ya) && (yv < yb);
-                const int y = a.reverse ? H - 1 - yv : yv;
+                const int yv = FOLD ? 2 * ra - 1 + (j - sa.pad) : ra - 1 + j;
+                const bool emit = FOLD ? (j >= sa.pad && yv >= 2 * ya && yv < 2 * yb) : (yv >= ya && yv < yb);
+                const int y = a.reverse ? (FOLD ? 2 * H : H) - 1 - yv : yv;
                 const uint32_t slot = ring_slot<S>(v);
                 const uint32_t col = slot * NOUT;
                 const uint32_t col2 = (S + slot) * NOUT;
                 const bool dual = slot < 2;
-                const size_t pix = (static_cast<size_t>(valid ? n : 0) * a.H + y) * a.W + (valid ? x : 0);
+                const size_t pix = FOLD ? (static_cast<size_t>(valid ? n : 0) * 2 * a.H + y) * 2 * a.W + (valid ? 2 * x + phb : 0)
+                                        : (static_cast<size_t>(valid ? n : 0) * a.H + y) * a.W + (valid ? x : 0);
                 bool waited = false;
+                uint8_t* tileR = tile_base;
+                uint8_t* tile16 = tile_base;
 #pragma unroll 1
                 for (int h = 0; h < NSUB; ++h) {
                     const int ls = slice * NSUB + h;
@@ -484,9 +523,11 @@
                         }
                     }
                     PROF_ADD(p_math, p_tm);
-                    uint8_t* const tileR = tile_base + ((two_bufs && (pass & 1u)) ? buf_bytes : 0);
-                    uint8_t* const tile16 = tileR + (a.has_outf ? kTileFBytes : 0);
-                    if (staged) {
+                    const bool stage_here = staged && (!FOLD || h == 0);
+                    const bool store_here = staged && (!FOLD || h == NSUB - 1);
+                    if (stage_here) {
+                        tileR = tile_base + ((two_bufs && (pass & 1u)) ? buf_bytes : 0);
+                        tile16 = tileR + (a.has_outf ? kTileFBytes : 0);
                         PROF_T0(p_t);
                         if (lead_warp) { if (two_bufs) tma_store_wait_read1(); else tma_store_wait_read(); }
                         named_bar_sync(1 + gi, 128);
@@ -590,19 +631,27 @@
                                 pk[i] = pack_f16x2_sat(val[2 * i], val[2 * i + 1]);
                             }
                         }
-                        uint4* dst = reinterpret_cast<uint4*>(tile16 + m * (SUBW * 2));
-#pragma unroll
-                        for (int i = 0; i < SUBW / 8; ++i) dst[i] = make_uint4(pk[4 * i], pk[4 * i + 1], pk[4 * i + 2], pk[4 * i + 3]);
-                    }
-                    if (staged) {
+                        uint4* dst = reinterpret_cast<uint4*>(tile16 + m * (TILE16W * 2));
+                        if (FOLD) {
+#pragma unroll
+                            for (int i = 0; i < SUBW / 8; ++i)
+                                dst[(h * (SUBW / 8) + i) ^ (m & 7)] = make_uint4(pk[4 * i], pk[4 * i + 1], pk[4 * i + 2], pk[4 * i + 3]);
+                        } else {
+#pragma unroll
+                            for (int i = 0; i < SUBW / 8; ++i) dst[i] = make_uint4(pk[4 * i], pk[4 * i + 1], pk[4 * i + 2], pk[4 * i + 3]);
+                        }
+                    }
+                    if (store_here) {
                         fence_proxy_async_smem();
                         named_bar_sync(1 + gi, 128);
                         if (lead_warp) {
                             if (elect_one()) {
                                 if (use_outf) tma_store_4d(&tmapOF, tileR, a.outf_choff + ls * SUBW, x0, y, n0);
                                 if (use_o16) {
-                                    const int c0 = a.out16_choff + (a.out16_slice_fixed ? 0 : ls * SUBW);
-                                    if (!a.out16_up2) {
+                                    const int c0 = a.out16_choff + (a.out16_slice_fixed || FOLD ? 0 : ls * SUBW);
+                                    if (FOLD) {
+                                        tma_store_5d(&tmapO16, tile16, c0, phb, x0, y, n0);
+                                    } else if (!a.out16_up2) {
                                         tma_store_4d(&tmapO16, tile16, c0, x0, y, n0);
                                     } else {
 #pragma unroll
@@ -634,7 +683,7 @@
                     }
                 }
             }
-            v0 += n_acc;
+            v0 += sa.n_acc;
             g += yb - ya;
         }
         if (lead_warp) tma_store_wait_all();
@@ -654,7 +703,7 @@
 
 bool conv3x3_pair_plan_smem(ConvArgs* a, int nout) {
     const int subw = nout == 64 ? 32 : nout;
-    const int wbytes = a->nchunks * 3 * (3 * nout / 2) * 128;
+    const int wbytes = pair_wbytes(*a, nout);
     int nepi = a->has_outf ? 2 : 3;
     const char* env = getenv("RESR_CONV_NEPI");
     if (env) nepi = atoi(env);
@@ -665,10 +714,10 @@
         a->nepi = nepi;
         for (int bufs = env_bufs == 2 ? 2 : 1; bufs >= 1; --bufs) {
             a->epi_bufs = bufs;
-            const int fixed = 1024 + wbytes + nepi * epi_group_bytes_pair(*a, subw) + kMiscBytes;
+            const int fixed = 1024 + wbytes + nepi * epi_group_bytes_pair(*a, a->in_up2 ? nout : subw) + kMiscBytes;
             int ns = (kSmemMax - fixed) / kStageBytes;
             if (ns > kMaxStages) ns = kMaxStages;
-            if ((bufs == 2 && ns >= 6) || (bufs == 1 && (ns >= 4 || nepi == 1))) {
+            if ((bufs == 2 && ns >= (a->in_up2 ? 4 : 6)) || (bufs == 1 && (ns >= 4 || nepi == 1))) {
                 a->nstages = ns;
                 return ns >= 2;
             }
@@ -676,11 +725,11 @@
     }
 }
 
-template <int NOUT>
+template <int NOUT, bool FOLD>
 static cudaError_t launch_pair_t(const ConvMaps& maps, const ConvArgs& args, dim3 grid, int threads, cudaStream_t stream) {
     static PerDevice<bool> attr;
     if (!attr.cur()) {
-        cudaError_t e = cudaFuncSetAttribute(conv3x3_pair_kernel<NOUT>, cudaFuncAttributeMaxDynamicSharedMemorySize, kSmemMax);
+        cudaError_t e = cudaFuncSetAttribute(conv3x3_pair_kernel<NOUT, FOLD>, cudaFuncAttributeMaxDynamicSharedMemorySize, kSmemMax);
         if (e != cudaSuccess) return e;
         attr.cur() = true;
     }
@@ -699,17 +748,21 @@
     at[1].val.clusterDim.z = 1;
     cfg.attrs = at;
     cfg.numAttrs = 2;
-    return cudaLaunchKernelEx(&cfg, conv3x3_pair_kernel<NOUT>, maps.a, maps.o16, maps.of, args);
+    return cudaLaunchKernelEx(&cfg, conv3x3_pair_kernel<NOUT, FOLD>, maps.a, maps.o16, maps.of, args);
 }
 
 cudaError_t conv3x3_pair_launch(const ConvMaps& maps, const ConvArgs& args_in, int nout, int nslices, int num_sms,
                                 cudaStream_t stream) {
     ConvArgs args = args_in;
     const int subw = nout == 64 ? 32 : nout;
-    const int wbytes = args.nchunks * 3 * (3 * nout / 2) * 128;
-    const int smem = 1024 + wbytes + args.nstages * kStageBytes + args.nepi * epi_group_bytes_pair(args, subw) + kMiscBytes;
+    const int wbytes = pair_wbytes(args, nout);
+    const int smem = 1024 + wbytes + args.nstages * kStageBytes + args.nepi * epi_group_bytes_pair(args, args.in_up2 ? nout : subw) +
+                     kMiscBytes;
     if (args.nstages < 2 || args.nepi < 1 || args.nepi > 3 || smem > kSmemMax) return cudaErrorInvalidConfiguration;
     if (args.has_outf && subw != 32) return cudaErrorInvalidConfiguration;
+    if (args.in_up2 && (nout != 64 || nslices != 2 || !args.has_out16 || args.out16_up2 || args.has_outf || args.out_nchw ||
+                        args.out_u8 || args.out_nchw_raw || args.mask16))
+        return cudaErrorInvalidConfiguration;
     const long long ncg2 = (args.ncg + 1) / 2;
     args.rows_total_pair = ncg2 * args.H;
     long long npairs = (num_sms / 2) / nslices;
@@ -721,9 +774,10 @@
     if (args.tail_ksteps != 1 && args.tail_ksteps != 2 && args.tail_ksteps != 4) args.tail_ksteps = 4;
     const dim3 grid(static_cast<unsigned>(2 * npairs), static_cast<unsigned>(nslices), 1);
     const int threads = 128 + 128 * args.nepi;
-    if (nout == 64) return launch_pair_t<64>(maps, args, grid, threads, stream);
-    if (nout == 32) return launch_pair_t<32>(maps, args, grid, threads, stream);
-    if (nout == 16) return launch_pair_t<16>(maps, args, grid, threads, stream);
+    if (args.in_up2) return launch_pair_t<64, true>(maps, args, grid, threads, stream);
+    if (nout == 64) return launch_pair_t<64, false>(maps, args, grid, threads, stream);
+    if (nout == 32) return launch_pair_t<32, false>(maps, args, grid, threads, stream);
+    if (nout == 16) return launch_pair_t<16, false>(maps, args, grid, threads, stream);
     return cudaErrorInvalidValue;
 }
 
@@ -750,6 +804,14 @@
     cfg->pair = 0;
     cfg->nout = pack_nout;
     cfg->nslices = pack_nslices;
+    if (a->in_up2) {
+        if (!env_pair || a->ncg < 2 || pack_nout != 32 || pack_nslices != 2) return false;
+        ConvArgs t = *a;
+        if (!conv3x3_pair_plan_smem(&t, 64)) return false;
+        *a = t;
+        cfg->pair = 1; cfg->nout = 64; cfg->nslices = 2;
+        return true;
+    }
     const long long pair_rows = static_cast<long long>((a->ncg + 1) / 2) * a->H;
     const bool big_enough = pair_rows >= 6 * 74 || env_pair == 2;
     if (env_pair && a->ncg >= 2 && big_enough) {
diff --git a/real_esrgan-pytorch_b200/csrc/conv3x3_tc.cu b/real_esrgan-pytorch_b200/csrc/conv3x3_tc.cu
--- a/real_esrgan-pytorch_b200/csrc/conv3x3_tc.cu
+++ b/real_esrgan-pytorch_b200/csrc/conv3x3_tc.cu
@@ -651,7 +651,8 @@
                                        static_cast<cuuint64_t>(2 * W) * C * 2, static_cast<cuuint64_t>(2 * H) * 2 * W * C * 2};
         const cuuint32_t box[5] = {static_cast<cuuint32_t>(nout), 1, static_cast<cuuint32_t>(BW), 1, static_cast<cuuint32_t>(BN)};
         r = enc(out, CU_TENSOR_MAP_DATA_TYPE_UINT16, 5, const_cast<void*>(base), dims, strides, box, estr,
-                CU_TENSOR_MAP_INTERLEAVE_NONE, CU_TENSOR_MAP_SWIZZLE_NONE, CU_TENSOR_MAP_L2_PROMOTION_NONE,
+                CU_TENSOR_MAP_INTERLEAVE_NONE, nout == 64 ? CU_TENSOR_MAP_SWIZZLE_128B : CU_TENSOR_MAP_SWIZZLE_NONE,
+                CU_TENSOR_MAP_L2_PROMOTION_NONE,
                 CU_TENSOR_MAP_FLOAT_OOB_FILL_NONE);
     }
     return r == CUDA_SUCCESS ? 0 : static_cast<int>(r);
diff --git a/real_esrgan-pytorch_b200/csrc/gen_internal.cuh b/real_esrgan-pytorch_b200/csrc/gen_internal.cuh
--- a/real_esrgan-pytorch_b200/csrc/gen_internal.cuh
+++ b/real_esrgan-pytorch_b200/csrc/gen_internal.cuh
@@ -19,7 +19,11 @@
     size_t wt_off;
     int t_nslices;
     int t_nchunks;
+    size_t wf_off;
 };
+
+static const int kConvUp1 = 347, kConvUp2 = 348;
+inline size_t fold_bytes(int nchunks) { return static_cast<size_t>(2) * nchunks * 2 * 256 * 128; }
 
 static const int kNumConvs = 351;
 static const int kNumRRDB = 23;
@@ -60,6 +64,10 @@
             c[k].t_nchunks = (c[k].cout + 63) / 64;
             c[k].wt_off = wt;
             wt += static_cast<size_t>(c[k].t_nslices) * c[k].t_nchunks * 3 * 96 * 128;
+        }
+        for (int k = kConvUp1; k <= kConvUp2; ++k) {
+            c[k].wf_off = w;
+            w += fold_bytes(c[k].nchunks);
         }
         n_params = p;
         pack_bytes = w;
diff --git a/real_esrgan-pytorch_b200/csrc/generator.cu b/real_esrgan-pytorch_b200/csrc/generator.cu
--- a/real_esrgan-pytorch_b200/csrc/generator.cu
+++ b/real_esrgan-pytorch_b200/csrc/generator.cu
@@ -54,6 +54,44 @@
         for (size_t i = first; i < static_cast<size_t>(nb); i += stride) bp[i] = (i < static_cast<size_t>(cout) && bias) ? bias[i] : 0.f;
 }
 
+__device__ __forceinline__ void pack_fold_body(const float* __restrict__ w, uint16_t* __restrict__ wp, int cin, int cout, int nchunks,
+                                               int fmt, size_t first, size_t stride) {
+    const size_t total = static_cast<size_t>(2) * nchunks * 2 * 256 * 64;
+    for (size_t idx = first; idx < total; idx += stride) {
+        const int k = static_cast<int>(idx & 63);
+        unsigned t = static_cast<unsigned>(idx >> 6);
+        const int n = t % 256;
+        t /= 256;
+        const int tap = t % 2;
+        t /= 2;
+        const int chunk = t % nchunks;
+        const int b = static_cast<int>(t / nchunks);
+        const int co = n & 63, f = n >> 6, gx = b + 2 * tap;
+        const int ci = chunk * 64 + k;
+        const int lo_y = f == 3 ? 2 : f >> 1, hi_y = f == 0 ? 0 : (f + 2) >> 1;
+        const int lo_x = gx == 3 ? 2 : gx >> 1, hi_x = gx == 0 ? 0 : (gx + 2) >> 1;
+        float v = 0.f;
+        if (co < cout && ci < cin)
+            for (int ky = lo_y; ky <= hi_y; ++ky)
+                for (int kx = lo_x; kx <= hi_x; ++kx) v = __fadd_rn(v, w[((static_cast<size_t>(co) * cin + ci) * 3 + ky) * 3 + kx]);
+        uint16_t bits;
+        if (fmt == 1) {
+            __nv_bfloat16 h = __float2bfloat16_rn(v);
+            bits = *reinterpret_cast<uint16_t*>(&h);
+        } else {
+            __half h = __float2half_rn(v);
+            bits = *reinterpret_cast<uint16_t*>(&h);
+        }
+        const size_t tile = ((static_cast<size_t>(b) * nchunks + chunk) * 2 + tap) * 256 * 64;
+        wp[tile + static_cast<size_t>(n) * 64 + ((((k >> 3) ^ (n & 7)) << 3) | (k & 7))] = bits;
+    }
+}
+
+__global__ void pack_fold_kernel(const float* __restrict__ w, uint16_t* __restrict__ wp, int cin, int cout, int nchunks, int fmt) {
+    pack_fold_body(w, wp, cin, cout, nchunks, fmt, blockIdx.x * static_cast<size_t>(blockDim.x) + threadIdx.x,
+                   static_cast<size_t>(gridDim.x) * blockDim.x);
+}
+
 __global__ void pack_conv_kernel(const float* __restrict__ w, const float* __restrict__ bias, uint16_t* __restrict__ wp,
                                  float* __restrict__ bp, int cin, int cout, int nout, int nslices, int nchunks, int fmt,
                                  int transposed) {
@@ -64,12 +102,18 @@
 struct PackJob {
     unsigned long long p_off, w_off, b_off;
     int cin, cout, nout, nslices, nchunks, fmt;
+    int fold;
 };
 __global__ void __launch_bounds__(256) pack_all_kernel(const float* __restrict__ flat, const PackJob* __restrict__ jobs,
                                                        uint8_t* __restrict__ wpack, float* __restrict__ bias, int transposed) {
     const PackJob j = jobs[blockIdx.y];
     const float* w = flat + j.p_off;
     const float* b = w + static_cast<size_t>(j.cout) * j.cin * 9;
+    if (j.fold) {
+        pack_fold_body(w, reinterpret_cast<uint16_t*>(wpack + j.w_off), j.cin, j.cout, j.nchunks, j.fmt,
+                       blockIdx.x * static_cast<size_t>(blockDim.x) + threadIdx.x, static_cast<size_t>(gridDim.x) * blockDim.x);
+        return;
+    }
     pack_conv_body(w, transposed ? nullptr : b, reinterpret_cast<uint16_t*>(wpack + j.w_off), transposed ? nullptr : bias + j.b_off,
                    j.cin, j.cout, j.nout, j.nslices, j.nchunks, j.fmt, transposed,
                    blockIdx.x * static_cast<size_t>(blockDim.x) + threadIdx.x, static_cast<size_t>(gridDim.x) * blockDim.x);
@@ -202,8 +246,9 @@
 int launch_pack_all(resr_generator* g, const float* flat, int transposed, cudaStream_t s) {
     const Table& T = table();
     PackJob** slot = reinterpret_cast<PackJob**>(transposed ? &g->pack_jobs_t : &g->pack_jobs);
+    const int njobs = transposed ? kNumConvs : kNumConvs + 2;
     if (!*slot) {
-        std::vector<PackJob> h(kNumConvs);
+        std::vector<PackJob> h(njobs);
         for (int k = 0; k < kNumConvs; ++k) {
             const ConvSpec& c = T.c[k];
             PackJob& j = h[k];
@@ -215,13 +260,19 @@
             } else {
                 j.w_off = c.wt_off; j.b_off = 0; j.nout = 32; j.nslices = c.t_nslices; j.nchunks = c.t_nchunks; j.fmt = 1;
             }
-        }
-        if (cudaMalloc(slot, kNumConvs * sizeof(PackJob)) != cudaSuccess) return -1;
-        cudaMemcpyAsync(*slot, h.data(), kNumConvs * sizeof(PackJob), cudaMemcpyHostToDevice, s);
+            j.fold = 0;
+        }
+        for (int k = kNumConvs; k < njobs; ++k) {
+            h[k] = h[kConvUp1 + (k - kNumConvs)];
+            h[k].w_off = T.c[kConvUp1 + (k - kNumConvs)].wf_off;
+            h[k].fold = 1;
+        }
+        if (cudaMalloc(slot, njobs * sizeof(PackJob)) != cudaSuccess) return -1;
+        cudaMemcpyAsync(*slot, h.data(), njobs * sizeof(PackJob), cudaMemcpyHostToDevice, s);
         cudaStreamSynchronize(s);
     }
     const int first = transposed ? 1 : 0;
-    pack_all_kernel<<<dim3(24, kNumConvs - first), 256, 0, s>>>(flat, *slot + first, transposed ? g->wpack_t : g->wpack, g->bias,
+    pack_all_kernel<<<dim3(24, njobs - first), 256, 0, s>>>(flat, *slot + first, transposed ? g->wpack_t : g->wpack, g->bias,
                                                                 transposed);
     return cudaGetLastError() == cudaSuccess ? 0 : -2;
 }
@@ -239,6 +290,21 @@
 }
 
 static size_t align_up(size_t v, size_t a) { return (v + a - 1) / a * a; }
+
+static bool fold_upsample(int N, int H, int W, int s) {
+    if (s == 0 && !fold_upsample(N, H, W, 1)) return false;
+    ConvArgs a;
+    memset(&a, 0, sizeof(a));
+    a.N = N; a.H = H << s; a.W = W << s;
+    conv3x3_pick_tile(a.W, &a.BW, &a.BN);
+    a.nxs = (a.W + a.BW - 1) / a.BW;
+    a.ncg = ((N + a.BN - 1) / a.BN) * a.nxs;
+    a.nchunks = 1;
+    a.has_out16 = 1;
+    a.in_up2 = 1;
+    ConvLaunchCfg cfg;
+    return conv3x3_choose(&a, 32, 2, &cfg);
+}
 
 struct WsLayout {
     size_t xin, c[3], f0, m[4], t1, t2, t3, t4, total;
@@ -376,25 +442,35 @@
             ++conv;
         }
     }
+    const bool fold[2] = {fold_upsample(N, H, W, 0), fold_upsample(N, H, W, 1)};
+    auto make_up_step = [&](int s, const void* in16, void* out16) {
+        Step st = make_step(conv, fold[s] ? s : s + 1, in16, 64);
+        st.a.lrelu = 1;
+        if (fold[s]) {
+            st.a.in_up2 = 1;
+            st.a.wpack = g->wpack + T.c[conv].wf_off;
+            st.a.has_out16 = 1; st.a.out16_fmt = prec == 1 ? 1 : 0;
+            map_rc |= conv3x3_make_tmap_out16(&st.maps.o16, out16, N, geo[s].H, geo[s].W, 64, 64, geo[s].BW, geo[s].BN, 1);
+        } else {
+            set_out16(st, s + 1, out16, 64, 0, 0, s == 0 && !fold[1]);
+        }
+        return st;
+    };
     {
         Step st = make_step(conv, 0, cbuf[0], 192);
         st.a.ep_mode = EP_SKIP;
         set_res1(st, F0);
-        set_out16(st, 0, t1, 64, 0, 0, 1);
+        set_out16(st, 0, t1, 64, 0, 0, fold[0] ? 0 : 1);
         push(st);
         ++conv;
     }
     {
-        Step st = make_step(conv, 1, t1, 64);
-        st.a.lrelu = 1;
-        set_out16(st, 1, t2, 64, 0, 0, 1);
+        Step st = make_up_step(0, t1, t2);
         push(st);
         ++conv;
     }
     {
-        Step st = make_step(conv, 2, t2, 64);
-        st.a.lrelu = 1;
-        set_out16(st, 2, t3, 64, 0, 0, 0);
+        Step st = make_up_step(1, t2, t3);
         push(st);
         ++conv;
     }
@@ -700,13 +776,18 @@
     const int nslices = (d->cout + nout - 1) / nout;
     const int nchunks = (d->cin + 63) / 64;
     if (nchunks * 64 > d->c_total) return set_error(RESR_E_INVALID, "c_total must cover cin rounded up to 64");
-    const size_t pack_bytes = static_cast<size_t>(nslices) * nchunks * 3 * (3 * nout) * 128;
+    if (d->in_up2 && (d->cout != 64 || !d->out16 || d->out16_up2 || d->outf || d->out_nchw))
+        return set_error(RESR_E_INVALID, "in_up2 needs cout = 64 and a plain 16-bit output only");
+    const size_t pack_bytes = d->in_up2 ? fold_bytes(nchunks) : static_cast<size_t>(nslices) * nchunks * 3 * (3 * nout) * 128;
     uint8_t* wp = nullptr;
     float* bp = nullptr;
     if (cudaMalloc(&wp, pack_bytes) != cudaSuccess || cudaMalloc(&bp, nslices * nout * 4) != cudaSuccess)
         return set_error(RESR_E_CUDA, "cudaMalloc failed");
     launch_pack_conv(d->weight, d->bias, reinterpret_cast<uint16_t*>(wp), bp, d->cin, d->cout, nout, nslices, nchunks,
                      d->fmt_in, 0, s);
+    if (d->in_up2)
+        pack_fold_kernel<<<grid_for(pack_bytes / 2, 256), 256, 0, s>>>(d->weight, reinterpret_cast<uint16_t*>(wp), d->cin, d->cout,
+                                                                          nchunks, d->fmt_in);
     cudaStreamSynchronize(s);
     ConvArgs a;
     ConvMaps maps;
@@ -727,8 +808,10 @@
     int rc = conv3x3_make_tmap_act(&maps.a, d->in16, d->n, d->h, d->w, d->c_total, a.mode, a.BW, a.BN, d->cin);
     if (d->out16) {
         a.has_out16 = 1; a.out16_fmt = d->out16_fmt; a.out16_choff = d->out16_choff; a.out16_up2 = d->out16_up2;
-        rc |= conv3x3_make_tmap_out16(&maps.o16, d->out16, d->n, d->h, d->w, d->out16_cstride, nout, a.BW, a.BN, d->out16_up2);
-    }
+        rc |= conv3x3_make_tmap_out16(&maps.o16, d->out16, d->n, d->h, d->w, d->out16_cstride, d->in_up2 ? 64 : nout, a.BW, a.BN,
+                                      d->out16_up2 || d->in_up2);
+    }
+    a.in_up2 = d->in_up2 ? 1 : 0;
     if (d->outf) {
         a.has_outf = 1; a.outf_choff = d->outf_choff; a.outf = static_cast<float*>(d->outf); a.outf_cstride = d->outf_cstride;
         rc |= conv3x3_make_tmap_f32(&maps.of, d->outf, d->n, d->h, d->w, d->outf_cstride, a.BW, a.BN);
@@ -742,7 +825,15 @@
     a.dbg = d->dbg;
     a.dbg_flags = d->dbg_flags;
     ConvLaunchCfg cfg;
-    if (!conv3x3_choose(&a, nout, nslices, &cfg)) rc |= 1 << 20;
+    if (!conv3x3_choose(&a, nout, nslices, &cfg)) {
+        if (a.in_up2) {
+            cudaStreamSynchronize(s);
+            cudaFree(wp);
+            cudaFree(bp);
+            return set_error(RESR_E_INVALID, "in_up2 runs on the CTA-pair kernel only (two column groups, pair policy != 0)");
+        }
+        rc |= 1 << 20;
+    }
     if (nout == 16 && (d->out16 || d->outf || d->res1)) rc |= 1 << 21;
     cudaError_t e = cudaSuccess;
     if (rc == 0) e = conv3x3_run(maps, a, cfg, sms, s);
```

After: 25.24, median of 6. 2.5% higher.
